# TheCacophonyProject/classifier-pipeline

Measured on AMD Instinct MI355X. Metric: CPTV frames/s end-to-end (track+classify) at 160x120, higher is better.
Workload: dtype u16/i32 track stage (f32 normalise, f64 gates); f32 crop/tile; f32 CNN (stride-1 3x3 convs of stages 2-4 (+ the stride-2 one): two fp16 planes per operand rounded to nearest (11 + 11 significand bits), power-of-two range scaling, 3 fp16 MFMAs per K step, device-side rerun in the exact split if an ac

## Files before the change

classifier-pipeline_amd/csrc/cpx_api.cpp:

```cpp
#include <hip/hip_runtime.h>

#include <algorithm>
#include <cmath>
#include <cstdio>
#include <cstdlib>
#include <cstring>
#include <new>
#include <string>
#include <vector>

#include "cpx_internal.h"
#include "cpx_schedule_core.h"

static_assert(sizeof(cpx_component) == 32, "cpx_component layout is part of the ABI");
static_assert(sizeof(cpx_frame_info) == 80, "cpx_frame_info layout is part of the ABI");
static_assert(sizeof(cpx_frame_meta) == 24, "cpx_frame_meta layout is part of the ABI");
static_assert(sizeof(cpx_config) == 48, "cpx_config layout is part of the ABI");
static_assert(sizeof(cpx_region_ref) == 24 && sizeof(cpx_track_limits) == 32 && sizeof(cpx_crop_req) == 32,
              "classification request layouts are part of the ABI");
static_assert(sizeof(cpx_filter_params) == 72 && sizeof(cpx_track_summary) == 120,
              "end-of-clip layouts are part of the ABI");
static_assert(sizeof(cpx_region) == 56, "cpx_region layout is part of the ABI");
static_assert(sizeof(cpx_track_record) == 32, "cpx_track_record layout is part of the ABI");
static_assert(sizeof(cpx_track_params) == 120, "cpx_track_params layout is part of the ABI");

namespace {

struct WsLayout {
  size_t bg, wsum, kcnt, filt, cstate, u8, carry, bgavg, big, total;
};

WsLayout ws_layout(const cpx_config& c, int B, bool need_filt_state) {
  const size_t P = (size_t)c.width * c.height;
  WsLayout l{};
  size_t off = 0;
  l.bg = off;
  off = align_up(off + (size_t)B * 2 * P * sizeof(uint16_t), 256);
  l.wsum = off;
  off = align_up(off + (size_t)B * P * sizeof(uint32_t), 256);
  l.kcnt = off;
  off = align_up(off + (size_t)B * P * sizeof(uint16_t), 256);
  l.filt = off;
  if (need_filt_state) off = align_up(off + (size_t)B * 2 * P * sizeof(float), 256);
  l.cstate = off;
  off = align_up(off + (size_t)B * sizeof(cpx::ClipState), 256);
  l.u8 = off;
  off = align_up(off + (size_t)B * 2 * P, 256);
  l.carry = off;
  off = align_up(off + (size_t)B * 2 * sizeof(cpx::FrameCarry), 256);
  l.bgavg = off;
  off = align_up(off + (size_t)B * sizeof(double), 256);
  l.big = off;
  if (c.max_components > cpx::track_lds_components())
    off = align_up(off + (size_t)B * 9 * c.max_components * sizeof(uint32_t), 256);
  l.total = off;
  return l;
}

int build_schedule(cpx_handle* h, const int32_t* clip_offsets, const cpx_frame_meta* meta, int B, cpx::Schedule* sc) {
  switch (cpx::schedule_build(clip_offsets, meta, B, h->cfg.max_frames, sc)) {
    case cpx::SchedError::EmptyClip: return fail(h, CPX_ERR_INVALID, "empty clip in batch");
    case cpx::SchedError::TooLong: return fail(h, CPX_ERR_INVALID, "clip longer than max_frames");
    case cpx::SchedError::Ok: break;
  }
  return CPX_OK;
}

int upload_schedule(cpx_handle* h, const cpx::Schedule& sc, int B, cpx::SchedLayout* sl) {
  const std::vector<int> flat = cpx::schedule_flatten(sc, B);
  *sl = cpx::SchedLayout::of(B, (int)sc.proc_idx.size());
  if (int rc = h->sched.grow(h, flat.size() * sizeof(int), "schedule hipMalloc")) return rc;
  CPX_HIP(h, hipMemcpyAsync(h->sched.p, flat.data(), flat.size() * sizeof(int), hipMemcpyHostToDevice, h->stream));
  CPX_HIP(h, hipStreamSynchronize(h->stream));
  return CPX_OK;
}

}

extern "C" {

int cpx_abi_version(void) { return CPX_ABI_VERSION; }

int cpx_create(int device_id, const cpx_config* cfg, cpx_handle** out) {
  if (!cfg || !out) return CPX_ERR_INVALID;
  *out = nullptr;
  int ndev = 0;
  if (hipGetDeviceCount(&ndev) != hipSuccess || ndev <= 0) return CPX_ERR_NO_DEVICE;
  if (device_id < 0 || device_id >= ndev) return CPX_ERR_INVALID;
  const int W = cfg->width, H = cfg->height;
  if (W <= 0 || H <= 0 || (W % 8) != 0 || W >= 192 || W * H > cpx::track_max_pixels() || H < 5 || W < 8)
    return CPX_ERR_UNSUPPORTED;
  if (cfg->edge_pixels < 0 || 2 * cfg->edge_pixels >= std::min(W, H) || cfg->window < 1 ||
      cfg->max_components < 1 || cfg->max_frames < 1 || cfg->max_frames > 65534)
    return CPX_ERR_INVALID;
  cpx_handle* h = new (std::nothrow) cpx_handle();
  if (!h) return CPX_ERR_NOMEM;
  h->device = device_id;
  h->cfg = *cfg;
  if (hipSetDevice(device_id) != hipSuccess || hipStreamCreateWithFlags(&h->stream, hipStreamNonBlocking) != hipSuccess ||
      hipStreamCreateWithFlags(&h->stream2, hipStreamNonBlocking) != hipSuccess ||
      hipEventCreateWithFlags(&h->ev_median, hipEventDisableTiming) != hipSuccess ||
      hipEventCreate(&h->ev0) != hipSuccess || hipEventCreate(&h->ev1) != hipSuccess) {
    cpx_destroy(h);
    return CPX_ERR_HIP;
  }
  h->wtab_len = 65536;
  h->wtab_host.resize(h->wtab_len);
  std::vector<double>& wt = h->wtab_host;
  double w = 0.0;
  for (int k = 0; k < h->wtab_len; ++k) {
    wt[k] = w;
    w = w + cfg->weight_add;
  }
  if (cfg->denoise) {
    if (!cpx::nlm_supported(W, H)) {
      cpx_destroy(h);
      return CPX_ERR_UNSUPPORTED;
    }
    const int fixed_point_mult = (int)(2147483647LL / (21 * 21 * 255));
    std::vector<int> lut(64, 0);
    for (int a2 = 0; a2 < 64; ++a2) {
      const double wv = std::exp(-((double)a2 * (64.0 / 49.0)) / 9.0);
      const double wr = std::nearbyint((double)fixed_point_mult * wv);
      lut[a2] = (wr < 0.001 * fixed_point_mult) ? 0 : (int)wr;
    }
    if (lut[63] != 0 || h->nlm_lut_dev.grow(h, 64 * sizeof(int), "NLM weight table allocation") ||
        hipMemcpy(h->nlm_lut_dev.p, lut.data(), 64 * sizeof(int), hipMemcpyHostToDevice) != hipSuccess) {
      cpx_destroy(h);
      return CPX_ERR_HIP;
    }
  }
  std::vector<uint32_t> thr(h->wtab_len);
  for (int k = 0; k < h->wtab_len; ++k) {
    const double wk = wt[k], m = std::nearbyint(wk);
    const bool exact = (wk == m), near = !exact && std::fabs(wk - m) < 1e-6;
    double hi = near ? m + 1.0 : std::floor(wk) + 1.0;
    if (!(hi >= 0.0)) hi = 0.0;
    if (hi > 536870912.0) hi = 536870912.0;
    thr[k] = 2u * (uint32_t)hi - (near ? 1u : 0u);
  }
  if (h->wthr_dev.grow(h, thr.size() * sizeof(uint32_t), "threshold table allocation") ||
      hipMemcpy(h->wthr_dev.p, thr.data(), thr.size() * sizeof(uint32_t), hipMemcpyHostToDevice) != hipSuccess) {
    cpx_destroy(h);
    return CPX_ERR_HIP;
  }
  if (h->wtab_dev.grow(h, wt.size() * sizeof(double), "weight table allocation") ||
      hipMemcpy(h->wtab_dev.p, wt.data(), wt.size() * sizeof(double), hipMemcpyHostToDevice) != hipSuccess ||
      cpx::frame_kernel_attr_setup() != 0) {
    cpx_destroy(h);
    return CPX_ERR_HIP;
  }
  if (const char* env = std::getenv("CPX_TRACK_PACKED_STATE")) h->packed_state_ok = std::atoi(env) != 0;
  if (const char* env = std::getenv("CPX_CNN_FUSE_CONV1")) h->fuse_conv1 = std::atoi(env) != 0;
  if (const char* env = std::getenv("CPX_TRACK_PER_STEP")) h->track_per_step = std::atoi(env) != 0;
  if (const char* env = std::getenv("CPX_CNN_FUSE_SHORTCUT")) h->fuse_shortcut = std::atoi(env) != 0;
  if (const char* env = std::getenv("CPX_CNN_SHORTCUT_FP16")) h->shortcut_fp16 = std::atoi(env) != 0;
  if (const char* env = std::getenv("CPX_CNN_BLOCK_FUSION")) h->block_fusion = std::min(std::max(std::atoi(env), 0), 2);
  if (const char* env = std::getenv("CPX_CNN_MATH")) {
    if (!std::strcmp(env, "f32")) h->cnn_math = CPX_CNN_MATH_F32;
    else if (!std::strcmp(env, "bf16x3")) h->cnn_math = CPX_CNN_MATH_BF16X3;
    else if (!std::strcmp(env, "bf16x2")) h->cnn_math = CPX_CNN_MATH_BF16X2;
    else if (!std::strcmp(env, "fp16x2")) h->cnn_math = CPX_CNN_MATH_FP16X2;
  }
  *out = h;
  return CPX_OK;
}

static void release_buffers(cpx_handle* h, bool all) {
  for (DeviceBuffer* b : {&h->ws, &h->ws_assoc, &h->bf3_scratch, &h->cnn_arena, &h->graph_arena, &h->ir_scratch}) b->release();
  if (!all) return;
  for (DeviceBuffer* b : {&h->sched, &h->wtab_dev, &h->wthr_dev, &h->nlm_lut_dev, &h->cnn_ovf, &h->ir_bitmap}) b->release();
}

void cpx_destroy(cpx_handle* h) {
  if (!h) return;
  hipSetDevice(h->device);
  if (h->stream) hipStreamSynchronize(h->stream);
  for (cpx_cnn* c : h->cnns) cnn_free(c);
  h->cnns.clear();
  for (cpx_mog2* m : h->mog2s) mog2_free(m);
  h->mog2s.clear();
  for (cpx_graph* g : h->graphs) graph_free(g);
  h->graphs.clear();
  release_buffers(h, true);
  for (auto& e : h->conv_events) {
    hipEventDestroy(e.e0);
    hipEventDestroy(e.e1);
  }
  if (h->stream2) {
    hipStreamSynchronize(h->stream2);
    hipStreamDestroy(h->stream2);
  }
  if (h->ev_median) hipEventDestroy(h->ev_median);
  if (h->ev0) hipEventDestroy(h->ev0);
  if (h->ev1) hipEventDestroy(h->ev1);
  if (h->stream) hipStreamDestroy(h->stream);
  delete h;
}

const char* cpx_last_error(const cpx_handle* h) { return h ? h->err.c_str() : "null handle"; }

void* cpx_stream(cpx_handle* h) { return h ? (void*)h->stream : nullptr; }

static int join_medians(cpx_handle* h) {
  if (h->medians_pending) {
    h->medians_pending = false;
    CPX_HIP(h, hipStreamWaitEvent(h->stream, h->ev_median, 0));
  }
  return CPX_OK;
}

int cpx_join_medians(cpx_handle* h) {
  if (!h) return CPX_ERR_INVALID;
  return join_medians(h);
}

int cpx_release_memory(cpx_handle* h) {
  if (!h) return CPX_ERR_INVALID;
  CPX_ENTER(h);
  if (int rc = join_medians(h)) return rc;
  CPX_HIP(h, hipStreamSynchronize(h->stream));
  CPX_HIP(h, hipStreamSynchronize(h->stream2));
  release_buffers(h, false);
  h->last_B = 0;
  h->state_packed = false;
  return CPX_OK;
}

int cpx_synchronize(cpx_handle* h) {
  if (!h) return CPX_ERR_INVALID;
  if (int rc = join_medians(h)) return rc;
  CPX_HIP(h, hipStreamSynchronize(h->stream));
  return CPX_OK;
}

size_t cpx_track_workspace_bytes(const cpx_handle* h, int B, int total_frames) {
  if (!h || B <= 0) return 0;
  (void)total_frames;
  return ws_layout(h->cfg, B, true).total;
}

static int unpack_state(cpx_handle* h) {
  if (h->state_packed && h->ws.p && h->last_B > 0) {
    const WsLayout lp = ws_layout(h->cfg, h->last_B, h->stream_filt_state);
    char* base = h->ws.as<char>();
    cpx::launch_unpack_state((uint32_t*)(base + lp.wsum), (uint16_t*)(base + lp.kcnt),
                             (size_t)h->last_B * h->cfg.width * h->cfg.height, h->stream);
    CPX_HIP(h, hipGetLastError());
  }
  h->state_packed = false;
  return CPX_OK;
}

static int track_run(cpx_handle* h, const uint16_t* frames_dev, const int32_t* clip_offsets,
                     const cpx_frame_meta* meta, int B, int n_prev, cpx_component* comps_dev,
                     cpx_frame_info* info_dev, int32_t* labels_dev, float* filtered_dev,
                     float* background_dev, int flags) {
  CPX_ENTER(h);
  if (flags & ~(CPX_TRACK_KEEP_BACKGROUND | CPX_TRACK_FREEZE_ON_FFC | CPX_TRACK_FREEZE_BACKGROUND | CPX_TRACK_DEFER_MEDIANS))
    return fail(h, CPX_ERR_INVALID, "track: unknown flag");
  if (int jrc = join_medians(h)) return jrc;
  const bool defer_medians = (flags & CPX_TRACK_DEFER_MEDIANS) != 0;
  const cpx_config& c = h->cfg;
  cpx::Schedule sc;
  int rc = build_schedule(h, clip_offsets, meta, B, &sc);
  if (rc != CPX_OK) return rc;
  const int total = sc.total, max_proc = sc.max_proc;
  const bool resume = n_prev > 0;
  const int t_begin = cpx::processed_before(meta, n_prev);
  const bool need_filt = (filtered_dev == nullptr);
  const WsLayout l = ws_layout(c, B, need_filt);
  if (resume && (l.total > h->ws.bytes || need_filt != h->stream_filt_state))
    return fail(h, CPX_ERR_INVALID, "cpx_track_frame: the stream's workspace is gone (optional outputs changed?)");
  const bool keep = !resume && (flags & CPX_TRACK_KEEP_BACKGROUND);
  if (keep) {
    const bool have_prev = h->ws.p && h->last_B == B && need_filt == h->stream_filt_state && l.total <= h->ws.bytes;
    for (int b = 0; b < B && !have_prev; ++b)
      if (!h->staged_bg.count(b)) {
        h->staged_bg.clear();
        return fail(h, CPX_ERR_INVALID, "CPX_TRACK_KEEP_BACKGROUND: no background state for a clip (previous call had another batch size, and nothing staged; staged states dropped)");
      }
  }
  for (const auto& kv : h->staged_bg)
    if (kv.first >= B) {
      h->staged_bg.clear();
      return fail(h, CPX_ERR_INVALID, "cpx_set_background: staged clip index outside the batch (staged states dropped)");
    }
  if (resume || keep) {
    if (int urc = unpack_state(h)) return urc;
  }
  h->state_packed = false;
  h->stream_filt_state = need_filt;
  h->last_B = B;
  struct StateGuard {
    cpx_handle* h;
    bool armed = true;
    ~StateGuard() {
      if (armed) {
        h->last_B = 0;
        h->state_packed = false;
      }
    }
  } guard{h};
  if ((rc = h->ws.grow(h, l.total, "workspace hipMalloc"))) return rc;
  cpx::SchedLayout sl;
  rc = upload_schedule(h, sc, B, &sl);
  if (rc != CPX_OK) return rc;

  cpx::TrackArgs a{};
// ... 611 lines not shown
```

classifier-pipeline_amd/csrc/cpx_api_cnn.cpp:

```cpp
#include <hip/hip_runtime.h>

#include <algorithm>
#include <cmath>
#include <cstdio>
#include <cstdlib>
#include <new>
#include <utility>
#include <vector>

#include "cpx_internal.h"

static_assert(sizeof(cpx_wrresnet_block) == 56 && sizeof(cpx_wrresnet_params) == 1560,
              "cpx_wrresnet_params layout is part of the ABI");

struct cpx_cnn {
  cpx_handle* h = nullptr;
  cpx_wrresnet_params p{};
  std::vector<std::pair<const float*, void*>> split;
  float act_scale[3][CPX_WRRESNET_MAX_BLOCKS][2];
  float res_bound[3] = {0.0f, 0.0f, 0.0f};
  float sc_xscale[3] = {0.0f, 0.0f, 0.0f};
  void* sc_img[3] = {nullptr, nullptr, nullptr};
  double sc_wmax[3] = {-1.0, -1.0, -1.0};
  cpx_cnn() {
    for (auto& st : act_scale)
      for (auto& b : st) b[0] = b[1] = 1.0f;
  }
  const void* split_of(const float* w) const {
    for (const auto& e : split)
      if (e.first == w) return e.second;
    return nullptr;
  }
};

void cnn_free(cpx_cnn* c) {
  for (auto& e : c->split) hipFree(e.second);
  for (void* img : c->sc_img)
    if (img) hipFree(img);
  delete c;
}

struct conv_fuse {
  const float* in = nullptr;
  const float* w = nullptr;
  const float* bias = nullptr;
  int H = 0, W = 0, cin = 0, stride = 1;
  const void* planes = nullptr;
  float xscale = 0.0f;
};

static bool split_math(const cpx_handle* h) { return h->cnn_math != CPX_CNN_MATH_F32; }
struct conv_half {
  float act_scale = 1.0f;
  bool keep_flag = false;
  int word = 0;
  bool out_planes = false;
  float out_act_scale = 1.0f;
  bool in_planes = false;
  bool rerun_only = false;
};
constexpr int OVF_WORDS = 2 + 3 * CPX_WRRESNET_MAX_BLOCKS;
static int ensure_ovf_word(cpx_handle* h) {
  if (h->cnn_ovf.p) return CPX_OK;
  if (int rc = h->cnn_ovf.grow(h, OVF_WORDS * sizeof(int), "cpx_conv2d: overflow word allocation failed")) return rc;
  CPX_HIP(h, hipMemsetAsync(h->cnn_ovf.p, 0, OVF_WORDS * sizeof(int), h->stream));
  return CPX_OK;
}
static cpx::ConvArgs conv_shape(int N, int H, int W, int Cin, int Cout, int groups, int ksize, int stride, int pad_same) {
  cpx::ConvArgs a{};
  a.N = N; a.H = H; a.W = W; a.Cin = Cin; a.Cout = Cout; a.groups = groups; a.ksize = ksize; a.stride = stride;
  if (pad_same) {
    a.Ho = (H + stride - 1) / stride;
    a.Wo = (W + stride - 1) / stride;
    a.pad_top = std::max((a.Ho - 1) * stride + ksize - H, 0) / 2;
    a.pad_left = std::max((a.Wo - 1) * stride + ksize - W, 0) / 2;
  } else {
    a.Ho = (H - ksize) / stride + 1;
    a.Wo = (W - ksize) / stride + 1;
  }
  return a;
}
static cpx::ConvArgs conv_describe(const cpx_conv_desc& d, const conv_fuse* fuse = nullptr) {
  cpx::ConvArgs a = conv_shape(d.N, d.H, d.W, d.Cin, d.Cout, d.groups, d.ksize, d.stride, d.pad_same);
  a.relu = d.relu;
  a.in = d.in_dev; a.out = d.out_dev; a.weights = d.weights_dev;
  a.in_scale = d.in_scale_dev; a.in_shift = d.in_shift_dev;
  a.out_scale = d.out_scale_dev; a.out_shift = d.out_shift_dev; a.residual = d.residual_dev;
  if (fuse) {
    a.sc_in = fuse->in; a.sc_w = fuse->w; a.sc_bias = fuse->bias;
    a.sc_H = fuse->H; a.sc_W = fuse->W; a.sc_cin = fuse->cin; a.sc_stride = fuse->stride;
    a.sc_planes = fuse->planes; a.sc_xscale = fuse->xscale;
  }
  return a;
}

class ConvTimer {
 public:
  ConvTimer(cpx_handle* h, bool on) : h_(h) {
    if (!on) return;
    ok_ = hipEventCreate(&ev_.e0) == hipSuccess && hipEventCreate(&ev_.e1) == hipSuccess &&
          hipEventRecord(ev_.e0, h->stream) == hipSuccess;
  }
  ~ConvTimer() {
    if (ev_.e0) hipEventDestroy(ev_.e0);
    if (ev_.e1) hipEventDestroy(ev_.e1);
  }
  ConvTimer(const ConvTimer&) = delete;
  ConvTimer& operator=(const ConvTimer&) = delete;
  bool ok() const { return ok_; }
  int commit(int key, double flops) {
    if (!ev_.e0) return CPX_OK;
    CPX_HIP(h_, hipEventRecord(ev_.e1, h_->stream));
    ev_.key = key;
    ev_.flops = flops;
    h_->conv_events.push_back(ev_);
    ev_ = {};
    return CPX_OK;
  }

 private:
  cpx_handle* h_;
  cpx_handle::ConvEv ev_{};
  bool ok_ = true;
};

enum class ConvRoute {
  Float32,
  Split,
  Fp16Pair,
  RerunOnly,
};

static int conv_run(cpx_handle* h, const cpx_conv_desc* d, const void* split_weights, const conv_fuse* fuse = nullptr,
                    const conv_half* hf = nullptr) {
  if (!h) return CPX_ERR_INVALID;
  if (!d || !d->in_dev || !d->out_dev || !d->weights_dev) return fail(h, CPX_ERR_INVALID, "cpx_conv2d: null argument");
  if (d->N < 1 || d->H < 1 || d->W < 1 || d->groups < 1 || d->Cin % d->groups || d->Cout % d->groups ||
      d->ksize < 1 || d->stride < 1 || (d->in_scale_dev == nullptr) != (d->in_shift_dev == nullptr))
    return fail(h, CPX_ERR_INVALID, "cpx_conv2d: bad descriptor");
  CPX_ENTER(h);
  if (!d->pad_same && (d->H < d->ksize || d->W < d->ksize)) return fail(h, CPX_ERR_INVALID, "cpx_conv2d: input smaller than kernel");
  cpx::ConvArgs a = conv_describe(*d, fuse);
  const bool split = split_math(h) && cpx::conv_bf3_supported(a);
  if (fuse && (!split || a.out_scale || a.residual))
    return fail(h, CPX_ERR_INVALID, "conv_run: shortcut fusion needs the split-operand kernel, no output scale, no residual");
  if (split) a.planes = h->cnn_math == CPX_CNN_MATH_BF16X2 ? 2 : 3;
  const conv_half bare;
  const conv_half& k = hf ? *hf : bare;
  const bool fp16 = split && h->cnn_math == CPX_CNN_MATH_FP16X2;
  const bool aliased = a.out == a.residual || a.out == a.in;
  const bool half = fp16 && cpx::conv_bf3_two_planes(a) && !aliased;
  const bool planes_out = fp16 && k.out_planes;
  const ConvRoute route = k.rerun_only ? ConvRoute::RerunOnly
                          : !split ? ConvRoute::Float32
                          : (half || planes_out) ? ConvRoute::Fp16Pair
                                                 : ConvRoute::Split;
  ConvTimer timer(h, h->conv_timing && route != ConvRoute::RerunOnly);
  if (!timer.ok()) return fail(h, CPX_ERR_HIP, "cpx_conv2d: event creation failed");
  int* word = nullptr;
  if (route == ConvRoute::Fp16Pair || route == ConvRoute::RerunOnly) {
    if (int rc = ensure_ovf_word(h)) return rc;
    if (!k.keep_flag) CPX_HIP(h, hipMemsetAsync(h->cnn_ovf.p, 0, sizeof(int), h->stream));
    word = h->cnn_ovf.as<int>() + k.word;
  }
  if (split && !split_weights) {
    if (int rc = h->bf3_scratch.grow(h, cpx::conv_bf3_weight_bytes(a), "cpx_conv2d: weight scratch allocation failed"))
      return rc;
    cpx::launch_split_weights(a, h->bf3_scratch.p, h->stream);
    split_weights = h->bf3_scratch.p;
  }
  int rc = 0;
  if (route == ConvRoute::Fp16Pair) {
    cpx::ConvArgs first = a;
    if (half) {
      first.planes = 2;
      first.half = 1;
      first.act_scale = k.act_scale;
      first.act_unscale = 1.0f / first.act_scale;
      first.in_planes = k.in_planes;
    }
    first.ovf = word;
    if (planes_out) {
      first.out_planes = 1;
      first.out_act_scale = k.out_act_scale;
    }
    rc = cpx::launch_conv_bf3(first, split_weights, h->stream);
  }
  a.guard = word;
  if (split) {
    if (rc == 0) rc = cpx::launch_conv_bf3(a, split_weights, h->stream);
    if (rc == -3) {
      if (fuse) return fail(h, CPX_ERR_UNSUPPORTED, "conv_run: batch too large for the fused-shortcut kernel (split the call)");
      rc = cpx::launch_conv(a, h->stream);
    }
  } else {
    rc = cpx::launch_conv(a, h->stream);
  }
  if (int trc = timer.commit((a.Cin / a.groups) * 10000 + (a.Cout / a.groups) * 10 + a.stride + (a.ksize == 1 ? 5 : 0),
                             2.0 * a.N * a.Ho * a.Wo * a.Cout * (double)(a.Cin / a.groups) * a.ksize * a.ksize))
    return trc;
  if (rc == -2) return fail(h, CPX_ERR_UNSUPPORTED, "cpx_conv2d: no kernel for this (channels per group, stride, kernel size)");
  if (rc != 0) return fail(h, CPX_ERR_HIP, "cpx_conv2d: kernel configuration failed");
  CPX_HIP(h, hipGetLastError());
  return CPX_OK;
}

static bool conv_can_fuse(const cpx_handle* h, int f, int groups) {
  return split_math(h) && cpx::conv_bf3_supported(conv_shape(0, 0, 0, f, f, groups, 3, 1, 1));
}

enum class BlockForm {
  OneLaunch,
  PlanesPair,
  Separate,
};
enum class Shortcut {
  Identity,
  FusedIntoSecond,
  OwnLaunch,
};
enum class Conv1 {
  NotHere,
  InFront,
  InsideBlock,
};
enum class Fusion { None, Block, BlockAndConv1 };

struct BlockPlan {
  int k, st, d;
  int stride, H, W, Ho, Wo, c_in, f;
  int word;
  BlockForm form;
  Shortcut shortcut;
  bool shortcut_fp16;
  Conv1 conv1;
};

struct Forward {
  cpx_cnn* cnn;
  cpx_handle* h;
  const float* in;
  int N, H, W;
  float *act[2], *mid, *sc;
};

static cpx_conv_desc layer_desc(const Forward& fw, const float* in, float* out, const float* w, int H, int W, int cin, int cout,
                                int ksize, int stride, int same, int relu) {
  cpx_conv_desc d{};
  d.N = fw.N; d.H = H; d.W = W; d.Cin = cin; d.Cout = cout; d.groups = fw.cnn->p.groups; d.ksize = ksize; d.stride = stride;
  d.pad_same = same; d.relu = relu;
  d.in_dev = in; d.out_dev = out; d.weights_dev = w;
  return d;
}

struct BlockLayers {
  cpx_conv_desc a, sc, b;
  conv_fuse fuse;
};
static BlockLayers block_layers(const Forward& fw, const BlockPlan& bp) {
  const cpx_wrresnet_params& p = fw.cnn->p;
  const cpx_wrresnet_block& b = p.block[bp.st][bp.d];
  const float* cur = fw.act[bp.k & 1];
  BlockLayers l{};
  l.a = layer_desc(fw, cur, fw.mid, b.wa, bp.H, bp.W, bp.c_in, bp.f, 3, bp.stride, 1, 1);
  l.a.in_scale_dev = b.in_scale; l.a.in_shift_dev = b.in_shift; l.a.out_scale_dev = b.a_scale; l.a.out_shift_dev = b.a_shift;
  l.sc = layer_desc(fw, cur, fw.sc, p.shortcut_w[bp.st], bp.H, bp.W, bp.c_in, bp.f, 1, bp.stride, 0, 0);
  l.sc.out_shift_dev = p.shortcut_b[bp.st];
  l.fuse.in = cur; l.fuse.w = p.shortcut_w[bp.st]; l.fuse.bias = p.shortcut_b[bp.st];
  l.fuse.H = bp.H; l.fuse.W = bp.W; l.fuse.cin = bp.c_in; l.fuse.stride = bp.stride;
  if (bp.shortcut_fp16) {
    l.fuse.planes = fw.cnn->sc_img[bp.st];
    l.fuse.xscale = fw.cnn->sc_xscale[bp.st];
  }
  l.b = layer_desc(fw, fw.mid, fw.act[(bp.k + 1) & 1], b.wb, bp.Ho, bp.Wo, bp.f, bp.f, 3, 1, 1, 1);
  l.b.out_shift_dev = b.bb;
  l.b.residual_dev = bp.shortcut == Shortcut::Identity ? cur : bp.shortcut == Shortcut::OwnLaunch ? fw.sc : nullptr;
  return l;
}
static void block32_args(const Forward& fw, const BlockPlan& bp, cpx::ConvArgs* ca, cpx::ConvArgs* cb) {
  const BlockLayers l = block_layers(fw, bp);
  *ca = conv_describe(l.a);
  *cb = conv_describe(l.b, bp.shortcut == Shortcut::FusedIntoSecond ? &l.fuse : nullptr);
  cpx::ConvArgs* both[2] = {ca, cb};
  for (int i = 0; i < 2; ++i) {
    both[i]->planes = 2;
    both[i]->half = 1;
    both[i]->ovf = fw.h->cnn_ovf.as<int>() + bp.word;
    both[i]->act_scale = fw.cnn->act_scale[bp.st][bp.d][i];
    both[i]->act_unscale = 1.0f / both[i]->act_scale;
  }
  if (bp.conv1 == Conv1::InsideBlock) {
    ca->c1_in = fw.in; ca->c1_w = fw.cnn->p.conv1_w; ca->c1_b = fw.cnn->p.conv1_b;
  }
}

static BlockPlan plan_block(const Forward& fw, int k, int H, int W, Fusion most) {
  const cpx_handle* h = fw.h;
  const cpx_cnn* cnn = fw.cnn;
  const cpx_wrresnet_params& p = cnn->p;
  const int g = p.groups;
  BlockPlan bp{};
  bp.k = k; bp.st = k / p.blocks_per_stage; bp.d = k % p.blocks_per_stage;
  const cpx_wrresnet_block& b = p.block[bp.st][bp.d];
  bp.stride = bp.d == 0 ? bp.st + 1 : 1;
  bp.c_in = p.filters[bp.d == 0 ? bp.st : bp.st + 1];
  bp.f = p.filters[bp.st + 1];
  const cpx::ConvArgs first = conv_shape(fw.N, H, W, bp.c_in, bp.f, g, 3, bp.stride, 1);
  const cpx::ConvArgs second = conv_shape(fw.N, first.Ho, first.Wo, bp.f, bp.f, g, 3, 1, 1);
  bp.H = H; bp.W = W; bp.Ho = first.Ho; bp.Wo = first.Wo;
  bp.word = 2 + k;
  const bool fp16 = h->cnn_math == CPX_CNN_MATH_FP16X2, whole_groups = bp.c_in % g == 0 && bp.f % g == 0;
  bp.shortcut = bp.d != 0 ? Shortcut::Identity
                : (h->fuse_shortcut && conv_can_fuse(h, bp.f, g) && (bp.c_in / g) % 4 == 0) ? Shortcut::FusedIntoSecond
                                                                                          : Shortcut::OwnLaunch;
  bp.shortcut_fp16 = bp.shortcut == Shortcut::FusedIntoSecond && fp16 && h->shortcut_fp16 && cnn->sc_xscale[bp.st] > 0.0f &&
                     cnn->sc_img[bp.st] != nullptr;
  const bool first8 = bp.d == 0 && bp.stride == 1 && bp.c_in / g == 8 && h->block_fusion >= 2 && h->fuse_shortcut;
  bool one_launch = most != Fusion::None && fp16 && h->block_fusion && bp.stride == 1 &&
                    ((bp.d != 0 && bp.c_in == bp.f) || first8) && b.in_scale && cnn->split_of(b.wa) && cnn->split_of(b.wb) &&
                    whole_groups;
  if (one_launch) {
    cpx::ConvArgs ca, cb;
    block32_args(fw, bp, &ca, &cb);
    one_launch = cpx::conv_block32_supported(ca, cb);
  }
  const bool c1_inside = one_launch && most == Fusion::BlockAndConv1 && k == 0 && first8 && h->fuse_conv1 && g == 2 &&
                         p.in_channels == 2 && p.filters[0] == 16;
  bp.conv1 = k != 0 ? Conv1::NotHere : c1_inside ? Conv1::InsideBlock : Conv1::InFront;
  const bool planes = fp16 && whole_groups && cpx::conv_bf3_can_store_planes(first) && cpx::conv_bf3_two_planes(second) &&
                      cpx::conv_bf3_can_load_planes(second);
  bp.form = one_launch ? BlockForm::OneLaunch : planes ? BlockForm::PlanesPair : BlockForm::Separate;
  return bp;
}

static int run_layer(const Forward& fw, const cpx_conv_desc& d, const conv_half& hf, const conv_fuse* fuse = nullptr) {
  return conv_run(fw.h, &d, fw.cnn->split_of(d.weights_dev), fuse, &hf);
}
static conv_half forward_half(int word, bool rerun_only) {
  conv_half hf;
  hf.keep_flag = true;
  hf.word = word;
  hf.rerun_only = rerun_only;
  return hf;
}

static int run_conv1(const Forward& fw, const conv_half& hf) {
  const cpx_wrresnet_params& p = fw.cnn->p;
  cpx_conv_desc d = layer_desc(fw, fw.in, fw.act[0], p.conv1_w, fw.H, fw.W, p.in_channels, p.filters[0], 3, 1, 1, 0);
  d.out_shift_dev = p.conv1_b;
  return run_layer(fw, d, hf);
}

static int run_layers(const Forward& fw, const BlockPlan& bp, bool planes, bool rerun_only) {
  const BlockLayers l = block_layers(fw, bp);
  const float* act_scale = fw.cnn->act_scale[bp.st][bp.d];
  const conv_half hf = forward_half(bp.word, rerun_only);
  conv_half ha = hf, hb = hf;
  ha.act_scale = act_scale[0];
  ha.out_planes = planes;
  ha.out_act_scale = act_scale[1];
  hb.act_scale = act_scale[1];
  hb.in_planes = planes;
  if (int rc = run_layer(fw, l.a, ha)) return rc;
  if (bp.shortcut == Shortcut::OwnLaunch)
    if (int rc = run_layer(fw, l.sc, hf)) return rc;
  return run_layer(fw, l.b, hb, bp.shortcut == Shortcut::FusedIntoSecond ? &l.fuse : nullptr);
}

static int run_one_launch(const Forward& fw, const BlockPlan& bp, int* declined) {
  cpx_handle* h = fw.h;
  const cpx_wrresnet_params& p = fw.cnn->p;
  const cpx_wrresnet_block& b = p.block[bp.st][bp.d];
  const int g = p.groups;
  cpx::ConvArgs ca, cb;
  block32_args(fw, bp, &ca, &cb);
  ConvTimer timer(h, h->conv_timing);
  if (!timer.ok()) return fail(h, CPX_ERR_HIP, "cpx_cnn_forward: event creation failed");
  *declined = cpx::launch_conv_block32(ca, cb, fw.cnn->split_of(b.wa), fw.cnn->split_of(b.wb), h->stream);
  if (*declined) return CPX_OK;
  double flops = 2.0 * fw.N * bp.H * bp.W * bp.f * ((double)(bp.c_in / g) + (double)(bp.f / g)) * 9;
  if (bp.conv1 == Conv1::InsideBlock) flops += 2.0 * fw.N * bp.H * bp.W * bp.c_in * (double)(p.in_channels / g) * 9;
  if (int rc = timer.commit((bp.c_in / g) * 10000 + 32 * 10 + 4, flops)) return rc;
  if (bp.conv1 == Conv1::InsideBlock)
    if (int rc = run_conv1(fw, forward_half(bp.word, true))) return rc;
  return run_layers(fw, bp, false, true);
}

static int downgrade(const Forward& fw, BlockPlan* bp, int declined) {
  if (bp->conv1 == Conv1::InsideBlock) {
    *bp = plan_block(fw, bp->k, bp->H, bp->W, Fusion::Block);
    return run_conv1(fw, forward_half(0, false));
  }
  if (declined != -2 && declined != -3) return fail(fw.h, CPX_ERR_HIP, "cpx_cnn_forward: block kernel configuration failed");
  *bp = plan_block(fw, bp->k, bp->H, bp->W, Fusion::None);
  return CPX_OK;
}

static int run_block(const Forward& fw, BlockPlan bp) {
  if (bp.conv1 == Conv1::InFront)
    if (int rc = run_conv1(fw, forward_half(0, false))) return rc;
  while (bp.form == BlockForm::OneLaunch) {
    int declined = 0;
    if (int rc = run_one_launch(fw, bp, &declined)) return rc;
    if (!declined) return CPX_OK;
    if (int rc = downgrade(fw, &bp, declined)) return rc;
  }
  return run_layers(fw, bp, bp.form == BlockForm::PlanesPair, false);
}

static int update_shortcut_images(cpx_cnn* cnn) {
  cpx_handle* h = cnn->h;
  const cpx_wrresnet_params& p = cnn->p;
  CPX_ENTER(h);
  for (int st = 0; st < 3; ++st) {
    cnn->sc_xscale[st] = 0.0f;
    const int g = p.groups, c_in = p.filters[st], f = p.filters[st + 1];
    if (!(cnn->res_bound[st] > 0.0f) || c_in % g || f % g) continue;
    cpx::ConvArgs second = conv_shape(0, 0, 0, f, f, g, 3, 1, 1);
    second.weights = p.block[st][0].wb;
    const void* wimg = cnn->split_of(second.weights);
    if (!wimg || !cpx::conv_shortcut_planes_layer(second, c_in / g)) continue;
    const int cin_g = c_in / g, cout_g = f / g;
    const float* w_scale_dev = cpx::conv_bf3_weight_scales(second, wimg);
    if (cnn->sc_wmax[st] < 0.0) {
      std::vector<float> ws((size_t)f), w((size_t)g * cin_g * cout_g);
      CPX_HIP(h, hipStreamSynchronize(h->stream));
      CPX_HIP(h, hipMemcpy(ws.data(), w_scale_dev, ws.size() * sizeof(float), hipMemcpyDeviceToHost));
      CPX_HIP(h, hipMemcpy(w.data(), p.shortcut_w[st], w.size() * sizeof(float), hipMemcpyDeviceToHost));
      double m = 0.0;
      for (int gi = 0; gi < g; ++gi)
        for (int k = 0; k < cin_g; ++k)
          for (int c = 0; c < cout_g; ++c)
            m = std::max(m, std::fabs((double)w[((size_t)gi * cin_g + k) * cout_g + c]) * ws[gi * cout_g + c]);
      cnn->sc_wmax[st] = m;
    }
    const float act_scale = cnn->act_scale[st][0][1];
    const double wmax = cnn->sc_wmax[st] * act_scale;
    float sx = 0.0f;
    if (!cpx_cnn_shortcut_scale(cnn->res_bound[st], (float)wmax, &sx)) continue;
    if (!cnn->sc_img[st] && hipMalloc(&cnn->sc_img[st], cpx::conv_shortcut_image_bytes(g, cin_g, cout_g)) != hipSuccess) {
      (void)hipGetLastError();
      cnn->sc_img[st] = nullptr;
      return fail(h, CPX_ERR_NOMEM, "cpx_cnn_set_residual_bounds: shortcut image allocation failed");
    }
    cpx::launch_split_shortcut(p.shortcut_w[st], cnn->sc_img[st], g, cin_g, cout_g, w_scale_dev, act_scale / sx, h->stream);
    CPX_HIP(h, hipGetLastError());
    cnn->sc_xscale[st] = sx;
  }
  return CPX_OK;
}

static int cnn_forward(cpx_cnn* cnn, const float* in_dev, int N, int H, int W, float* logits_dev, float* probs_dev,
                       float* const* taps, int* ovf_out) {
  cpx_handle* h = cnn->h;
  CPX_ENTER(h);
  const cpx_wrresnet_params& p = cnn->p;
  if (h->cnn_math == CPX_CNN_MATH_FP16X2) {
    const int rco = ensure_ovf_word(h);
    if (rco != CPX_OK) return rco;
    CPX_HIP(h, hipMemsetAsync(h->cnn_ovf.as<int>() + 2, 0, (OVF_WORDS - 2) * sizeof(int), h->stream));
  }
  size_t biggest = 0;
  {
    int hh = H, ww = W;
    biggest = (size_t)N * hh * ww * p.filters[0];
    for (int st = 0; st < 3; ++st) {
      const int s = st + 1;
      hh = (hh + s - 1) / s;
      ww = (ww + s - 1) / s;
      biggest = std::max(biggest, (size_t)N * hh * ww * p.filters[st + 1]);
    }
  }
  biggest = align_up(biggest, 64);
  if (int rc = h->cnn_arena.grow(h, 4 * biggest * sizeof(float), "cpx_cnn_forward: activation hipMalloc")) return rc;
  float* const arena = h->cnn_arena.as<float>();
  const Forward fw{cnn, h, in_dev, N, H, W, {arena, arena + biggest}, arena + 2 * biggest, arena + 3 * biggest};
  const int n_blocks = 3 * p.blocks_per_stage;
  BlockPlan plan[3 * CPX_WRRESNET_MAX_BLOCKS];
  int hh = H, ww = W;
  for (int k = 0; k < n_blocks; ++k) {
    plan[k] = plan_block(fw, k, hh, ww, Fusion::BlockAndConv1);
    hh = plan[k].Ho;
    ww = plan[k].Wo;
  }
  for (int k = 0; k < n_blocks; ++k) {
    if (int brc = run_block(fw, plan[k])) return brc;
    if (taps)
      CPX_HIP(h, hipMemcpyAsync(taps[k], fw.act[(k + 1) & 1], (size_t)N * plan[k].Ho * plan[k].Wo * plan[k].f * sizeof(float),
                                hipMemcpyDeviceToDevice, h->stream));
  }
  const float* cur = fw.act[n_blocks & 1];
  const int c_in = plan[n_blocks - 1].f;
  cpx_head_desc hd{};
  hd.N = N; hd.HW = hh * ww; hd.C = c_in; hd.L = p.n_labels;
  hd.n_hidden = p.n_hidden;
  hd.activation = p.activation;
  for (int k = 0; k < p.n_hidden; ++k) {
    hd.hidden_sizes[k] = p.hidden_sizes[k];
    hd.hidden_w_dev[k] = p.hidden_w[k];
    hd.hidden_b_dev[k] = p.hidden_b[k];
  }
  hd.in_dev = cur; hd.bn_scale_dev = p.final_scale; hd.bn_shift_dev = p.final_shift;
  hd.dense_w_dev = p.dense_w; hd.dense_b_dev = p.dense_b; hd.logits_dev = logits_dev; hd.probs_dev = probs_dev;
  int rc = cpx_cnn_head_ex(h, &hd);
  if (rc == CPX_OK && h->cnn_math == CPX_CNN_MATH_FP16X2)
    cpx::launch_count_overflow(h->cnn_ovf.as<int>(), 3 * p.blocks_per_stage, h->stream);
  if (rc == CPX_OK && ovf_out) {
    const size_t bytes = (size_t)3 * p.blocks_per_stage * sizeof(int);
    if (h->cnn_math == CPX_CNN_MATH_FP16X2)
      CPX_HIP(h, hipMemcpyAsync(ovf_out, h->cnn_ovf.as<int>() + 2, bytes, hipMemcpyDeviceToDevice, h->stream));
    else
      CPX_HIP(h, hipMemsetAsync(ovf_out, 0, bytes, h->stream));
  }
  if (rc == CPX_OK && h->cnn_math == CPX_CNN_MATH_FP16X2 && std::getenv("CPX_CNN_DEBUG_OVF")) {
    int words[OVF_WORDS];
    if (hipStreamSynchronize(h->stream) == hipSuccess &&
        hipMemcpy(words, h->cnn_ovf.p, sizeof(words), hipMemcpyDeviceToHost) == hipSuccess && words[0]) {
      std::fprintf(stderr, "cpx_cnn_forward: N = %d, fp16 overflow in blocks", N);
      for (int k = 0; k < 3 * p.blocks_per_stage; ++k)
        if (words[2 + k]) std::fprintf(stderr, " %d.%d", k / p.blocks_per_stage + 2, k % p.blocks_per_stage);
      std::fprintf(stderr, "\n");
    }
  }
  return rc;
}

extern "C" {

int cpx_conv2d(cpx_handle* h, const cpx_conv_desc* d) { return conv_run(h, d, nullptr); }

int cpx_set_cnn_math(cpx_handle* h, int mode) {
  if (!h) return CPX_ERR_INVALID;
  if (mode != CPX_CNN_MATH_F32 && mode != CPX_CNN_MATH_BF16X3 && mode != CPX_CNN_MATH_BF16X2 && mode != CPX_CNN_MATH_FP16X2)
    return fail(h, CPX_ERR_INVALID, "cpx_set_cnn_math: unknown mode");
  h->cnn_math = mode;
  return CPX_OK;
}
int cpx_get_cnn_math(const cpx_handle* h) { return h ? h->cnn_math : CPX_ERR_INVALID; }

int cpx_cnn_overflow_forwards(cpx_handle* h, int* count, int reset) {
  if (!h) return CPX_ERR_INVALID;
  if (!count) return fail(h, CPX_ERR_INVALID, "cpx_cnn_overflow_forwards: null argument");
  CPX_ENTER(h);
  *count = 0;
  if (!h->cnn_ovf.p) return CPX_OK;
  CPX_HIP(h, hipStreamSynchronize(h->stream));
  CPX_HIP(h, hipMemcpy(count, h->cnn_ovf.as<int>() + 1, sizeof(int), hipMemcpyDeviceToHost));
  if (reset) CPX_HIP(h, hipMemset(h->cnn_ovf.as<int>() + 1, 0, sizeof(int)));
  return CPX_OK;
}

int cpx_cnn_last_overflow(cpx_handle* h, int* overflowed) {
  if (!h) return CPX_ERR_INVALID;
  if (!overflowed) return fail(h, CPX_ERR_INVALID, "cpx_cnn_last_overflow: null argument");
  CPX_ENTER(h);
  *overflowed = 0;
  if (!h->cnn_ovf.p) return CPX_OK;
  CPX_HIP(h, hipStreamSynchronize(h->stream));
  CPX_HIP(h, hipMemcpy(overflowed, h->cnn_ovf.p, sizeof(int), hipMemcpyDeviceToHost));
  return CPX_OK;
}

int cpx_cnn_head_ex(cpx_handle* h, const cpx_head_desc* d) {
  if (!h) return CPX_ERR_INVALID;
  if (!d || !d->in_dev || !d->bn_scale_dev || !d->bn_shift_dev || !d->dense_w_dev || !d->dense_b_dev || !d->logits_dev ||
      d->N < 1 || d->HW < 1 || d->C < 1 || d->L < 1 || d->C > 8192 || d->L > 8192 || d->n_hidden < 0 ||
      d->n_hidden > CPX_HEAD_MAX_HIDDEN || (d->activation != CPX_HEAD_SIGMOID && d->activation != CPX_HEAD_SOFTMAX))
    return fail(h, CPX_ERR_INVALID, "cpx_cnn_head: bad argument");
  CPX_ENTER(h);
  cpx::HeadArgs a{};
  a.N = d->N; a.HW = d->HW; a.C = d->C; a.L = d->L;
  a.n_hidden = d->n_hidden;
  a.activation = d->activation;
  for (int k = 0; k < d->n_hidden; ++k) {
    if (!d->hidden_w_dev[k] || !d->hidden_b_dev[k] || d->hidden_sizes[k] < 1 || d->hidden_sizes[k] > 2048)
      return fail(h, CPX_ERR_INVALID, "cpx_cnn_head: bad hidden layer");
    a.hidden_sizes[k] = d->hidden_sizes[k];
    a.hidden_w[k] = d->hidden_w_dev[k];
    a.hidden_b[k] = d->hidden_b_dev[k];
  }
  a.in = d->in_dev; a.bn_scale = d->bn_scale_dev; a.bn_shift = d->bn_shift_dev;
  a.dense_w = d->dense_w_dev; a.dense_b = d->dense_b_dev; a.logits = d->logits_dev; a.probs = d->probs_dev;
  cpx::launch_head(a, h->stream);
  CPX_HIP(h, hipGetLastError());
  return CPX_OK;
}

int cpx_cnn_head(cpx_handle* h, const float* in_dev, int N, int HW, int C, const float* bn_scale_dev,
                 const float* bn_shift_dev, const float* dense_w_dev, const float* dense_b_dev, int L,
                 float* logits_dev, float* probs_dev) {
  if (!h) return CPX_ERR_INVALID;
  cpx_head_desc d{};
  d.N = N; d.HW = HW; d.C = C; d.L = L;
  d.n_hidden = 0;
  d.activation = CPX_HEAD_SIGMOID;
  d.in_dev = in_dev; d.bn_scale_dev = bn_scale_dev; d.bn_shift_dev = bn_shift_dev;
  d.dense_w_dev = dense_w_dev; d.dense_b_dev = dense_b_dev; d.logits_dev = logits_dev; d.probs_dev = probs_dev;
  return cpx_cnn_head_ex(h, &d);
}

int cpx_conv_timing_enable(cpx_handle* h, int enable) {
  if (!h) return CPX_ERR_INVALID;
  for (auto& e : h->conv_events) {
    hipEventDestroy(e.e0);
    hipEventDestroy(e.e1);
  }
  h->conv_events.clear();
  h->conv_timing = enable != 0;
  return CPX_OK;
}

int cpx_conv_timing_report(cpx_handle* h, cpx_conv_timing* out, int cap, int* n_out) {
  if (!h || !out || !n_out || cap < 1) return CPX_ERR_INVALID;
  CPX_HIP(h, hipStreamSynchronize(h->stream));
  int n = 0;
  for (auto& e : h->conv_events) {
    float ms = 0.f;
    CPX_HIP(h, hipEventElapsedTime(&ms, e.e0, e.e1));
    int i = 0;
    for (; i < n; ++i)
      if (out[i].key == e.key) break;
    if (i == n) {
      if (n == cap) return fail(h, CPX_ERR_OVERFLOW, "cpx_conv_timing_report: more kernel variants than capacity");
      out[n].key = e.key;
      out[n].launches = 0;
      out[n].total_ms = 0.0;
      out[n].flops = 0.0;
      n += 1;
    }
    out[i].launches += 1;
    out[i].total_ms += ms;
    out[i].flops += e.flops;
  }
  *n_out = n;
  return CPX_OK;
}
// ... 133 lines not shown
```

classifier-pipeline_amd/csrc/cpx_cnn_bf3.hip:

```cpp
#include <hip/hip_runtime.h>

#include <algorithm>
#include <cstdlib>
#include <type_traits>

#include "cpx_conv_layout_core.h"
#include "cpx_kernels.h"

namespace cpx {

namespace {

typedef float f32x16 __attribute__((ext_vector_type(16)));
typedef __bf16 bf16x8 __attribute__((ext_vector_type(8)));
typedef __bf16 bf16x2 __attribute__((ext_vector_type(2)));
typedef unsigned u32x4 __attribute__((ext_vector_type(4)));
typedef float f32x4 __attribute__((ext_vector_type(4)));

__device__ __forceinline__ unsigned pack2(float a, float b) {
  bf16x2 v = {(__bf16)a, (__bf16)b};
  return __builtin_bit_cast(unsigned, v);
}
template <typename T>
__device__ __forceinline__ const T* at_off(const T* base, unsigned bytes) {
// ... 372 lines not shown
      __builtin_amdgcn_fence(__ATOMIC_ACQUIRE, "wavefront");
      if (res_n) {
#pragma unroll
        for (int it = 0; it < 4; ++it) {
          const int f = it * 64 + lane;
          const int i = f >> 3, c4 = f & 7;
          const int oy = oy0 + (wset + m * WSETS) * TB + WR * wave + i / TW, ox = ox0 + i % TW;
          if (oy < a.Ho && ox < a.Wo) {
            float4 v = *reinterpret_cast<const float4*>(s_tile + i * 32 + 4 * c4);
            const int o = (int)pix_off(oy, ox, a.Wo, a.Cout) + ch0 + t * 32 + 4 * c4;
            const float4 rv = *reinterpret_cast<const float4*>(at_off(res_n, (unsigned)o << 2));
            v.x += rv.x; v.y += rv.y; v.z += rv.z; v.w += rv.w;
            if (a.relu) {
              v.x = relu_bits(v.x); v.y = relu_bits(v.y); v.z = relu_bits(v.z); v.w = relu_bits(v.w);
            }
            *reinterpret_cast<float4*>(at_off(out_n, (unsigned)o << 2)) = v;
          }
        }
      } else if (full_tile) {
        const unsigned lb = (pix_off(oy0 + (wset + m * WSETS) * TB + WR * wave, ox0 + (lane >> 3), a.Wo, a.Cout) +
                             (unsigned)(ch0 + t * 32 + 4 * (lane & 7))) << 2;
#pragma unroll
        for (int it = 0; it < 4; ++it) {
          float4 v = *reinterpret_cast<const float4*>(s_tile + (it * 64 + lane) * 4);
          const unsigned ub = (unsigned)((((it * 8) / TW) * a.Wo + ((it * 8) % TW)) * a.Cout) << 2;
          if (a.relu) {
            v.x = relu_bits(v.x); v.y = relu_bits(v.y); v.z = relu_bits(v.z); v.w = relu_bits(v.w);
          }
          if (a.out_planes) {
            const f32x4 vv = {v.x, v.y, v.z, v.w};
            if (max_abs4(vv) > F16_MAX) atomicOr(a.ovf, 1);
            *reinterpret_cast<u32x4*>(at_off(out_n, lb + ub)) = planes_of(vv);
          } else {
            *reinterpret_cast<float4*>(at_off(out_n, lb + ub)) = v;
          }
        }
      } else {
#pragma unroll
        for (int it = 0; it < 4; ++it) {
          const int f = it * 64 + lane;
          const int i = f >> 3, c4 = f & 7;
          const int oy = oy0 + (wset + m * WSETS) * TB + WR * wave + i / TW, ox = ox0 + i % TW;
          if (oy < a.Ho && ox < a.Wo) {
            float4 v = *reinterpret_cast<const float4*>(s_tile + i * 32 + 4 * c4);
            const int o = (int)pix_off(oy, ox, a.Wo, a.Cout) + ch0 + t * 32 + 4 * c4;
            if (a.relu) {
              v.x = relu_bits(v.x); v.y = relu_bits(v.y); v.z = relu_bits(v.z); v.w = relu_bits(v.w);
            }
            if (a.out_planes) {
              const f32x4 vv = {v.x, v.y, v.z, v.w};
              if (max_abs4(vv) > F16_MAX) atomicOr(a.ovf, 1);
              *reinterpret_cast<u32x4*>(at_off(out_n, (unsigned)o << 2)) = planes_of(vv);
            } else {
              *reinterpret_cast<float4*>(at_off(out_n, (unsigned)o << 2)) = v;
            }
          }
        }
      }
      if (m + 1 < NTM || t + 1 < NTN) {
        __builtin_amdgcn_fence(__ATOMIC_RELEASE, "wavefront");
        __builtin_amdgcn_wave_barrier();
        __builtin_amdgcn_fence(__ATOMIC_ACQUIRE, "wavefront");
      }
    }
  }
  BF3_TILE_LOOP_END
}

template <int NTN, int NPXC, int PL, bool H = false, bool PERSIST = false, int CT = 256, bool SC = false>
__global__ __launch_bounds__(CT) void conv_bf3flat_kernel(ConvArgs a, const uint4* __restrict__ wimg, TileDiv td) {
  constexpr int KS = 3, BAND = CT / 2;
  constexpr int COGW = 32 * NTN;
  static_assert(!H || PL == 2, "fp16 planes come in twos");
  static_assert(!SC || (H && !PERSIST && CT == 256 && 4 * 2 * 2 * BAND + 4 * 2 * 2 * COGW <= 2 * PL * NPXC + 18 * PL * COGW),
                "the shortcut's planes reuse the LDS of the patch and the weights");
  extern __shared__ __attribute__((aligned(16))) uint4 lds4[];
  BF3_ENTRY_GUARD(H)
  uint4* s_patch = lds4;
  uint4* s_w = lds4 + 2 * PL * NPXC;

  const int tid = threadIdx.x, lane = tid & 63, wave = tid >> 6;
  BF3_TILE_LOOP_BEGIN
  int bid = bid0;
  if (!PERSIST && (gridDim.x & 7) == 0) bid = (bid & 7) * (gridDim.x >> 3) + (bid >> 3);
  const int cin_g = a.Cin / a.groups, cout_g = a.Cout / a.groups;
  int q = div_magic(bid, td.m_nsplit);
  const int ns = bid - q * td.nsplit;
  bid = q;
  q = div_magic(bid, td.m_tx);
  const int ti = bid - q * td.tiles_x;
  const int n = q;
  const int g = blockIdx.y;
  const int M = a.Ho * a.Wo;
  const int p0 = ti * BAND;
  const int y_first = p0 / a.Wo, y_last = min(p0 + BAND - 1, M - 1) / a.Wo;
  const int PW = a.W + 2, PH = y_last - y_first + 3;
  const int npx = PH * PW;
  const int iy0 = y_first - a.pad_top, ix0 = -a.pad_left;
  const float* in_n = a.in + (size_t)n * a.H * a.W * a.Cin + (size_t)g * cin_g;
  const int nchunks = cin_g / KC;
  const uint4* wg = wimg + (size_t)g * nchunks * (18 * PL) * cout_g + (size_t)ns * COGW;

  const bool res_in_acc = a.residual != nullptr && a.out_scale == nullptr;
  f32x16 acc[NTN];
  if (res_in_acc) {
    const float* res_n = a.residual + (size_t)n * M * a.Cout + (g * cout_g + ns * COGW);
    const int rcol = lane & 31;
#pragma unroll
    for (int t = 0; t < NTN; ++t) {
      const float rs = H ? a.w_scale[g * cout_g + ns * COGW + t * 32 + rcol] * a.act_scale : 1.0f;
#pragma unroll
      for (int r = 0; r < 16; ++r) {
        const int i = (r & 3) + 8 * (r >> 2) + 4 * (lane >> 5);
        acc[t][r] = *at_off(res_n, (__umul24((unsigned)min(p0 + wave * 32 + i, M - 1), (unsigned)a.Cout) + (unsigned)(t * 32 + rcol)) << 2);
        if (H) acc[t][r] *= rs;
      }
    }
  } else {
#pragma unroll
    for (int t = 0; t < NTN; ++t)
#pragma unroll
      for (int r = 0; r < 16; ++r) acc[t][r] = 0.0f;
  }

  const int kh = lane >> 5;
  const int pl = min(p0 + wave * 32 + (lane & 31), M - 1);
  const int ly = pl / a.Wo, lx = pl - ly * a.Wo;
  const int a_base = kh * NPXC + (ly - y_first) * PW + lx;
  const int b_base = kh * COGW + (lane & 31);

  constexpr int NP = (2 * NPXC + CT - 1) / CT;
  constexpr int NW = 18 * PL * COGW;
  constexpr int NWI = (NW + CT - 1) / CT;
  const int my_h = tid & 1;
  int item_py[NP], item_px[NP], item_e[NP];
#pragma unroll
  for (int i = 0; i < NP; ++i) {
    const int item = min(tid + i * CT, 2 * npx - 1);
    const int px = item >> 1;
    item_py[i] = px / PW;
    item_px[i] = px - item_py[i] * PW;
    item_e[i] = my_h * NPXC + px;
  }
  f32x4 pre_p[NP][2];
  u32x4 pre_w[NWI];
  f32x4 psc[2], psh[2];
  for (int cc = -1; cc < nchunks; ++cc) {
    if (cc >= 0) {
      float vmax = 0.0f;
#pragma unroll
      for (int i = 0; i < NP; ++i) {
        const int iy = iy0 + item_py[i], ix = ix0 + item_px[i];
        const bool inside = iy >= 0 && iy < a.H && ix >= 0 && ix < a.W;
        float v[8];
#pragma unroll
        for (int j = 0; j < 8; ++j) v[j] = pre_p[i][j >> 2][j & 3];
        if (a.in_scale) {
#pragma unroll
          for (int j = 0; j < 8; ++j) v[j] = fmaxf(__fmaf_rn(v[j], psc[j >> 2][j & 3], psh[j >> 2][j & 3]), 0.0f);
        } else if (H) {
#pragma unroll
          for (int j = 0; j < 8; ++j) v[j] *= a.act_scale;
        }
#pragma unroll
        for (int j = 0; j < 8; ++j) v[j] = inside ? v[j] : 0.0f;
        if (H) {
#pragma unroll
          for (int j = 0; j < 8; j += 2) vmax = fmaxf(fmaxf(fabsf(v[j]), fabsf(v[j + 1])), vmax);
        }
        unsigned q0[4], q1[4], q2[4];
#pragma unroll
        for (int j = 0; j < 4; ++j) {
          if (PL == 3) split_pair(v[2 * j], v[2 * j + 1], q0[j], q1[j], q2[j]);
          else split2<H>(v[2 * j], v[2 * j + 1], q0[j], q1[j]);
        }
        u32x4* sp4 = reinterpret_cast<u32x4*>(s_patch);
        sp4[0 * 2 * NPXC + item_e[i]] = u32x4{q0[0], q0[1], q0[2], q0[3]};
        sp4[1 * 2 * NPXC + item_e[i]] = u32x4{q1[0], q1[1], q1[2], q1[3]};
        if (PL == 3) sp4[2 * 2 * NPXC + item_e[i]] = u32x4{q2[0], q2[1], q2[2], q2[3]};
      }
#pragma unroll
      for (int i = 0; i < NWI; ++i) {
        const int item = tid + i * CT;
        if (item < NW) reinterpret_cast<u32x4*>(s_w)[item] = pre_w[i];
      }
      if (H && vmax > F16_MAX) atomicOr(a.ovf, 1);
      __syncthreads();
    }
    if (cc + 1 < nchunks) {
      const int cn = (cc + 1) * KC;
      {
        const int ch = g * cin_g + cn;
        const float* scp = a.in_scale ? a.in_scale + ch : reinterpret_cast<const float*>(wimg);
        const float* shp = a.in_scale ? a.in_shift + ch : reinterpret_cast<const float*>(wimg);
        unsigned hoff = (unsigned)my_h << 5;
        asm volatile("" : "+v"(hoff));
        psc[0] = *reinterpret_cast<const f32x4*>(at_off(scp, hoff));
        psc[1] = *reinterpret_cast<const f32x4*>(at_off(scp, hoff + 16));
        psh[0] = *reinterpret_cast<const f32x4*>(at_off(shp, hoff));
        psh[1] = *reinterpret_cast<const f32x4*>(at_off(shp, hoff + 16));
        if (H) {
#pragma unroll
          for (int k = 0; k < 2; ++k) {
            psc[k] *= a.act_scale;
            psh[k] *= a.act_scale;
          }
        }
      }
#pragma unroll
      for (int i = 0; i < NP; ++i) {
        const int cy = min(max(iy0 + item_py[i], 0), a.H - 1), cx = min(max(ix0 + item_px[i], 0), a.W - 1);
        const unsigned soff = (pix_off(cy, cx, a.W, a.Cin) + (unsigned)(cn + 8 * my_h)) << 2;
        pre_p[i][0] = *reinterpret_cast<const f32x4*>(at_off(in_n, soff));
        pre_p[i][1] = *reinterpret_cast<const f32x4*>(at_off(in_n, soff + 16));
      }
      const u32x4* wc = reinterpret_cast<const u32x4*>(wg + (size_t)(cc + 1) * (18 * PL) * cout_g);
#pragma unroll
      for (int i = 0; i < NWI; ++i) {
        const int item = min(tid + i * CT, NW - 1);
        const int pth = item / COGW, col = item - pth * COGW;
        unsigned woff = (unsigned)(pth * cout_g + col) << 4;
        asm volatile("" : "+v"(woff));
        pre_w[i] = *at_off(wc, woff);
      }
    }
    if (cc >= 0) {
#pragma unroll
      for (int tap = 0; tap < KS * KS; ++tap) {
        const int ky = tap / KS, kx = tap - ky * KS;
        u32x4 av[PL], bv[NTN][PL];
#pragma unroll
        for (int p = 0; p < PL; ++p) {
          av[p] = __builtin_bit_cast(u32x4, s_patch[p * 2 * NPXC + a_base + ky * PW + kx]);
#pragma unroll
          for (int t = 0; t < NTN; ++t)
            bv[t][p] = __builtin_bit_cast(u32x4, s_w[(p * 9 + tap) * 2 * COGW + b_base + t * 32]);
        }
#pragma unroll
        for (int t = 0; t < NTN; ++t) {
          if (PL == 3) {
            acc[t] = mfma32<false>(av[1], bv[t][1], acc[t]);
            acc[t] = mfma32<false>(av[0], bv[t][PL - 1], acc[t]);
            acc[t] = mfma32<false>(av[PL - 1], bv[t][0], acc[t]);
          }
          acc[t] = mfma32<H>(av[0], bv[t][1], acc[t]);
          acc[t] = mfma32<H>(av[1], bv[t][0], acc[t]);
          acc[t] = mfma32<H>(av[0], bv[t][0], acc[t]);
        }
      }
      __syncthreads();
    }
  }

  if constexpr (SC) {
    uint4* s_x = lds4;
    uint4* s_scw = lds4 + 4 * 2 * 2 * BAND;
    {
      const int sp = min(p0 + (tid >> 1), M - 1);
      const int sy = sp / a.Wo, sxp = sp - sy * a.Wo;
      const float* src = a.sc_in + (((size_t)n * a.sc_H + sy * a.sc_stride) * a.sc_W + sxp * a.sc_stride) * a.sc_cin + g * 64 + 8 * my_h;
      f32x4 xv[4][2];
#pragma unroll
      for (int c = 0; c < 4; ++c) {
        xv[c][0] = *reinterpret_cast<const f32x4*>(src + 16 * c);
        xv[c][1] = *reinterpret_cast<const f32x4*>(src + 16 * c + 4);
      }
      u32x4 wv[4];
      const u32x4* scw = reinterpret_cast<const u32x4*>(a.sc_planes) + (size_t)g * 16 * cout_g + ns * COGW;
#pragma unroll
      for (int c = 0; c < 4; ++c) {
        const int col = tid & (COGW - 1), hh = (tid / COGW) & 1, pp = (tid / (2 * COGW)) & 1, j = 2 * c + hh;
        wv[c] = scw[(size_t)(((j >> 2) * 2 + pp) * 4 + (j & 3)) * cout_g + col];
      }
      float vmax = 0.0f;
#pragma unroll
      for (int c = 0; c < 4; ++c) {
        float v[8];
#pragma unroll
        for (int j = 0; j < 8; ++j) v[j] = xv[c][j >> 2][j & 3] * a.sc_xscale;
#pragma unroll
        for (int j = 0; j < 8; j += 2) vmax = fmaxf(fmaxf(fabsf(v[j]), fabsf(v[j + 1])), vmax);
        unsigned q0[4], q1[4];
#pragma unroll
        for (int j = 0; j < 4; ++j) split2<true>(v[2 * j], v[2 * j + 1], q0[j], q1[j]);
        u32x4* sx4 = reinterpret_cast<u32x4*>(s_x);
        sx4[((c * 2 + 0) * 2 + my_h) * BAND + (tid >> 1)] = u32x4{q0[0], q0[1], q0[2], q0[3]};
        sx4[((c * 2 + 1) * 2 + my_h) * BAND + (tid >> 1)] = u32x4{q1[0], q1[1], q1[2], q1[3]};
        reinterpret_cast<u32x4*>(s_scw)[c * (2 * 2 * COGW) + tid] = wv[c];
      }
      if (!(vmax <= F16_MAX)) atomicOr(a.ovf, 1);
    }
    __syncthreads();
#pragma unroll
    for (int c = 0; c < 4; ++c) {
      u32x4 av[2], bv[NTN][2];
#pragma unroll
      for (int p = 0; p < 2; ++p) {
        av[p] = __builtin_bit_cast(u32x4, s_x[((c * 2 + p) * 2 + kh) * BAND + wave * 32 + (lane & 31)]);
#pragma unroll
        for (int t = 0; t < NTN; ++t) bv[t][p] = __builtin_bit_cast(u32x4, s_scw[((c * 2 + p) * 2 + kh) * COGW + (lane & 31) + t * 32]);
      }
#pragma unroll
      for (int t = 0; t < NTN; ++t) {
        acc[t] = mfma32<true>(av[0], bv[t][1], acc[t]);
        acc[t] = mfma32<true>(av[1], bv[t][0], acc[t]);
        acc[t] = mfma32<true>(av[0], bv[t][0], acc[t]);
      }
    }
    __syncthreads();
  } else if (a.sc_in) {
    const int sc_cg = a.sc_cin / a.groups;
    const float* wsc = a.sc_w + (size_t)g * sc_cg * cout_g + ns * COGW + (lane & 31);
    const float* psc_in = a.sc_in + (((size_t)n * a.sc_H + ly * a.sc_stride) * a.sc_W + lx * a.sc_stride) * a.sc_cin +
                          g * sc_cg + kh;
    float ss[NTN];
#pragma unroll
    for (int t = 0; t < NTN; ++t) ss[t] = H ? a.w_scale[g * cout_g + ns * COGW + t * 32 + (lane & 31)] * a.act_scale : 1.0f;
    for (int k2 = 0; k2 < sc_cg; k2 += 2) {
      const float av = psc_in[k2];
#pragma unroll
      for (int t = 0; t < NTN; ++t) {
        float wv = wsc[(size_t)(k2 + kh) * cout_g + t * 32];
        if (H) wv *= ss[t];
        acc[t] = __builtin_amdgcn_mfma_f32_32x32x2f32(av, wv, acc[t], 0, 0, 0);
      }
    }
  }

  float* out_n = a.out + (size_t)n * M * a.Cout;
  const float* res_n = (a.residual && !res_in_acc) ? a.residual + (size_t)n * M * a.Cout : nullptr;
  float* s_tile = reinterpret_cast<float*>(lds4) + wave * (32 * 32);
  const int ch0 = g * cout_g + ns * COGW;
#pragma unroll
  for (int t = 0; t < NTN; ++t) {
    const int ch = ch0 + t * 32 + (lane & 31);
    float os = a.out_scale ? a.out_scale[ch] : 1.0f;
    if (H) os *= a.w_unscale[ch] * a.act_unscale;
    const float ob = (a.out_shift ? a.out_shift[ch] : 0.0f) + (a.sc_in && a.sc_bias ? a.sc_bias[ch] : 0.0f);
#pragma unroll
    for (int r = 0; r < 16; ++r) {
      const int i = (r & 3) + 8 * (r >> 2) + 4 * (lane >> 5);
      s_tile[i * 32 + (lane & 31)] = acc[t][r] * os + ob;
    }
    __builtin_amdgcn_fence(__ATOMIC_RELEASE, "wavefront");
    __builtin_amdgcn_wave_barrier();
    __builtin_amdgcn_fence(__ATOMIC_ACQUIRE, "wavefront");
    if (res_n) {
#pragma unroll
      for (int it = 0; it < 4; ++it) {
        const int f = it * 64 + lane;
        const int i = f >> 3, c4 = f & 7;
        const int p = p0 + wave * 32 + i;
        if (p < M) {
          f32x4 v = *reinterpret_cast<const f32x4*>(s_tile + i * 32 + 4 * c4);
          const int o = (int)__umul24((unsigned)p, (unsigned)a.Cout) + ch0 + t * 32 + 4 * c4;
          v += *reinterpret_cast<const f32x4*>(at_off(res_n, (unsigned)o << 2));
          if (a.relu) {
            v.x = relu_bits(v.x); v.y = relu_bits(v.y); v.z = relu_bits(v.z); v.w = relu_bits(v.w);
          }
          *reinterpret_cast<f32x4*>(at_off(out_n, (unsigned)o << 2)) = v;
        }
      }
    } else {
#pragma unroll
      for (int it = 0; it < 4; ++it) {
        const int f = it * 64 + lane;
        const int i = f >> 3, c4 = f & 7;
        const int p = p0 + wave * 32 + i;
        if (p < M) {
          f32x4 v = *reinterpret_cast<const f32x4*>(s_tile + i * 32 + 4 * c4);
          const int o = (int)__umul24((unsigned)p, (unsigned)a.Cout) + ch0 + t * 32 + 4 * c4;
          if (a.relu) {
            v.x = relu_bits(v.x); v.y = relu_bits(v.y); v.z = relu_bits(v.z); v.w = relu_bits(v.w);
          }
          *reinterpret_cast<f32x4*>(at_off(out_n, (unsigned)o << 2)) = v;
        }
      }
    }
    if (t + 1 < NTN) {
      __builtin_amdgcn_fence(__ATOMIC_RELEASE, "wavefront");
      __builtin_amdgcn_wave_barrier();
      __builtin_amdgcn_fence(__ATOMIC_ACQUIRE, "wavefront");
    }
  }
  BF3_TILE_LOOP_END
}

constexpr int KW = 32;
constexpr int W_TW = 16, W_TH = 16, W_PW = 18, W_NPX = 18 * 18;
constexpr int W_NPXP = 326;
constexpr int w_patch_entries(int planes) { return planes * 2 * W_NPXP * 2; }
constexpr int w_rows_resident(int planes) { return planes == 2 ? 3 : 1; }
constexpr int w_wsub_entries(int planes) { return w_rows_resident(planes) * planes * 3 * 4 * 32; }
template <bool WALK, bool LDSBN, int NH, int NG, int PL, bool H = false, bool PERSIST = false>
__global__ __launch_bounds__(512) __attribute__((amdgpu_waves_per_eu(4, 4))) void conv_bf3w_kernel(ConvArgs a, const uint4* __restrict__ wimg, TileDiv td) {
  static_assert(NG == 1 || (!WALK && !LDSBN && NH == 1), "the group walk is built for the one-slice, one-tile form");
  static_assert(PL == 2 || PL == 3, "two or three bf16 planes per operand");
  static_assert(!H || (PL == 2 && LDSBN), "fp16 planes come in twos (and with the BatchNorm parameters in LDS)");
  BF3_ENTRY_GUARD(H)
  constexpr int WR = w_rows_resident(PL);
  constexpr int W_PATCH = PL * 2 * W_NPXP * 2;
  constexpr int W_WROW = PL * 3 * 4 * 32;
  constexpr int W_WSUB = WR * W_WROW;
  constexpr int CT = 512;
  constexpr bool LAUNDER = WALK || NH > 1 || NG > 1 || PL == 2;
  extern __shared__ __attribute__((aligned(16))) uint4 lds4[];
  uint4* s_patch = lds4;
  uint4* s_w = lds4 + W_PATCH;

  const int tid = threadIdx.x, lane = tid & 63, wave = tid >> 6, i16 = lane & 15, q = lane >> 4;
  BF3_TILE_LOOP_BEGIN
  int bid = bid0;
  if (!PERSIST && (gridDim.x & 7) == 0) bid = (bid & 7) * (gridDim.x >> 3) + (bid >> 3);
  const int cin_g = a.Cin / a.groups, cout_g = a.Cout / a.groups;
  int qd = div_magic(bid, td.m_nsplit);
  const int ns = bid - qd * td.nsplit;
  bid = qd;
  qd = div_magic(bid, td.m_tx);
  const int txr = bid - qd * td.tiles_x;
  bid = qd;
  qd = div_magic(bid, td.m_ty);
  const int tyi = bid - qd * td.tiles_y;
  const int n = qd;
  const int g0 = blockIdx.y * NG;
  const int oy0 = tyi * W_TH;
  const int iy0 = oy0 - a.pad_top;
  const int run = WALK ? td.run : 1;
  const int tx_end = WALK ? min((txr + 1) * run, (a.Wo + W_TW - 1) / W_TW) : txr + 1;
  const float* in_n = a.in + (size_t)n * a.H * a.W * a.Cin;
  const int nch = cin_g / KW;
  const uint4* wg = wimg + (size_t)ns * (32 * NH);
  const int a_base = ((q >> 1) * W_NPXP + (2 * wave) * W_PW + i16) * 2 + (q & 1);
  const int b_base = q * 32 + i16;
  constexpr int NITEM = W_NPX * 8;
  constexpr int NP = (NITEM + CT - 1) / CT;
  constexpr int NWI = (W_WSUB + CT - 1) / CT;
  const int my_q8 = tid & 7;
  const int st_e2_0 = ((my_q8 >> 2) * W_NPXP + (tid >> 3)) * 4 + (my_q8 & 3);
  u32x4 pre_p[NP];
  u32x4 pre_w[NWI];
  f32x4* s_bn = reinterpret_cast<f32x4*>(lds4 + W_PATCH + W_WSUB);
#pragma clang diagnostic push
#pragma clang diagnostic ignored "-Wuninitialized"
  f32x4 psc_r, psh_r;
  if (LDSBN && a.in_scale) {
    if (tid < cin_g) {
      reinterpret_cast<float*>(s_bn)[tid] = a.in_scale[g0 * cin_g + tid] * (H ? a.act_scale : 1.0f);
      reinterpret_cast<float*>(s_bn)[cin_g + tid] = a.in_shift[g0 * cin_g + tid] * (H ? a.act_scale : 1.0f);
    }
    __syncthreads();
  }
#define BF3W_ISSUE_W(G_, C_, R_, HF_)                                                                     \
  {                                                                                                       \
    const uint4* wc = wg + (size_t)((((G_) * nch + (C_)) * 3 + (R_)) * (12 * PL)) * cout_g + (HF_) * 32;  \
    unsigned woff = (__umul24((unsigned)(tid >> 5), (unsigned)cout_g) + (unsigned)(tid & 31)) << 4;       \
    if (LAUNDER) asm volatile("" : "+v"(woff));                                                           \
    _Pragma("unroll") for (int i = 0; i < NWI; ++i) {                                                     \
       \
      const unsigned wo = (i == NWI - 1 && (W_WSUB % CT) != 0) ? (tid < (W_WSUB % CT) ? woff + ((unsigned)(16 * i * cout_g) << 4) : woff) : woff + ((unsigned)(16 * i * cout_g) << 4); \
      pre_w[i] = *at_off(reinterpret_cast<const u32x4*>(wc), wo);                                         \
    }                                                                                                     \
  }
#define BF3W_ISSUE_P(G_, C_, IX0_)                                                                        \
  {                                                                                                       \
    int t8 = tid >> 3;                                                                                    \
    if (LAUNDER) asm volatile("" : "+v"(t8));                                                             \
    int my_q8 = tid & 7;                                                                                  \
    if (LAUNDER) asm volatile("" : "+v"(my_q8));                                                          \
    if (!LDSBN) {                                                                                         \
      const int ch = (G_) * cin_g + (C_) * KW;                                                            \
      const float* scp = a.in_scale ? a.in_scale + ch : reinterpret_cast<const float*>(wimg);             \
      const float* shp = a.in_scale ? a.in_shift + ch : reinterpret_cast<const float*>(wimg);             \
      unsigned qoff = (unsigned)my_q8 << 4;                                                               \
      asm volatile("" : "+v"(qoff));                                                                      \
      psc_r = *reinterpret_cast<const f32x4*>(at_off(scp, qoff));                                         \
      psh_r = *reinterpret_cast<const f32x4*>(at_off(shp, qoff));                                         \
    }                                                                                                     \
    const unsigned coff = (unsigned)((G_) * cin_g + (C_) * KW + 4 * my_q8);                               \
    _Pragma("unroll") for (int i = 0; i < NP; ++i) {                                                      \
      const int px = min(t8 + 64 * i, W_NPX - 1);                                                         \
                                            \
      const int py = (int)(__umul24((unsigned)px, 3641u) >> 16), pxx = __mul24(py, -W_PW) + px;           \
      const int cy = min(max(iy0 + py, 0), a.H - 1), cx = min(max((IX0_) + pxx, 0), a.W - 1);             \
      pre_p[i] = *reinterpret_cast<const u32x4*>(at_off(in_n, (pix_off(cy, cx, a.W, a.Cin) + coff) << 2)); \
    }                                                                                                     \
  }
  BF3W_ISSUE_W(g0, 0, 0, 0)
  BF3W_ISSUE_P(g0, 0, txr * run * W_TW - a.pad_left)
  for (int txi = txr * run; txi < tx_end; ++txi) {
  const int ox0 = txi * W_TW, ix0 = ox0 - a.pad_left;
  const bool interior = iy0 >= 0 && iy0 + 18 <= a.H && ix0 >= 0 && ix0 + 18 <= a.W;
  const bool full_tile = oy0 + W_TH <= a.Ho && ox0 + W_TW <= a.Wo;

  int ch_l;
  unsigned opix[2];
  bool ovalid[2];
  auto out_pixels = [&](const int g) __attribute__((always_inline)) {
    int t = tid;
    if (LAUNDER) asm volatile("" : "+v"(t));
    const int i16_ = t & 15, q_ = (t >> 4) & 3, wave_ = t >> 6;
// ... 794 lines not shown
  }
}

__global__ __launch_bounds__(256) void weight_scales_kernel(const float* __restrict__ w, float* __restrict__ wscale,
                                                            float* __restrict__ wunscale, int groups, int rows, int cout_g) {
  const int idx = blockIdx.x * blockDim.x + threadIdx.x;
  if (idx >= groups * cout_g) return;
  const int g = idx / cout_g, col = idx - g * cout_g;
  float m = 0.0f;
  for (int r = 0; r < rows; ++r) m = fmaxf(m, fabsf(w[((size_t)g * rows + r) * cout_g + col]));
  int e = 0;
  if (m > 0.0f && m < 3.0e38f) (void)frexpf(m, &e);
  else e = 4;
  const int kw = min(max(4 - e, -100), 100);
  wscale[idx] = ldexpf(1.0f, kw);
  wunscale[idx] = ldexpf(1.0f, -kw);
}

__global__ __launch_bounds__(256) void split_weights8h_kernel(const float* __restrict__ w, uint4* __restrict__ out, int groups,
                                                              const float* __restrict__ wscale) {
  const size_t total = (size_t)groups * 3 * 4 * 32;
  for (size_t idx = (size_t)blockIdx.x * blockDim.x + threadIdx.x; idx < total; idx += (size_t)gridDim.x * blockDim.x) {
    const int col = (int)(idx & 31), qq = (int)((idx >> 5) & 3), t = (int)((idx >> 7) % 3), g = (int)(idx / 384);
    const int tap = 4 * t + qq;
    const float ws = wscale[g * 32 + col];
    float v[8];
#pragma unroll
    for (int j = 0; j < 8; ++j) v[j] = tap < 9 ? w[(((size_t)g * 9 + tap) * 8 + j) * 32 + col] * ws : 0.0f;
    uint4 p0, p1;
    split_pair2_h(v[0], v[1], p0.x, p1.x);
    split_pair2_h(v[2], v[3], p0.y, p1.y);
    split_pair2_h(v[4], v[5], p0.z, p1.z);
    split_pair2_h(v[6], v[7], p0.w, p1.w);
    const size_t base = (size_t)g * B8_WIMG;
    out[base + (size_t)(t * 2 + 0) * 128 + qq * 32 + col] = p0;
    out[base + (size_t)(t * 2 + 1) * 128 + qq * 32 + col] = p1;
  }
}

__global__ __launch_bounds__(256) void split_weights_kernel(const float* __restrict__ w, uint4* __restrict__ out, int groups,
                                                            int cin_g, int cout_g, int planes, const float* __restrict__ wscale) {
  const int nchunks = cin_g / KC;
  const size_t total = (size_t)groups * nchunks * 9 * 2 * cout_g;
  for (size_t idx = (size_t)blockIdx.x * blockDim.x + threadIdx.x; idx < total; idx += (size_t)gridDim.x * blockDim.x) {
    size_t r = idx;
    const int col = (int)(r % cout_g);
    r /= cout_g;
    const int h = (int)(r & 1);
    r >>= 1;
    const int tap = (int)(r % 9);
    r /= 9;
    const int chunk = (int)(r % nchunks);
    const int g = (int)(r / nchunks);
    float v[8];
#pragma unroll
    for (int j = 0; j < 8; ++j)
      v[j] = w[(((size_t)g * 9 + tap) * cin_g + chunk * KC + 8 * h + j) * cout_g + col];
    uint4 p0, p1, p2;
    if (wscale) {
      const float ws = wscale[g * cout_g + col];
      split_pair2_h(v[0] * ws, v[1] * ws, p0.x, p1.x);
      split_pair2_h(v[2] * ws, v[3] * ws, p0.y, p1.y);
      split_pair2_h(v[4] * ws, v[5] * ws, p0.z, p1.z);
      split_pair2_h(v[6] * ws, v[7] * ws, p0.w, p1.w);
    } else if (planes == 3) {
      split_pair(v[0], v[1], p0.x, p1.x, p2.x);
      split_pair(v[2], v[3], p0.y, p1.y, p2.y);
      split_pair(v[4], v[5], p0.z, p1.z, p2.z);
      split_pair(v[6], v[7], p0.w, p1.w, p2.w);
    } else {
      split_pair2(v[0], v[1], p0.x, p1.x);
      split_pair2(v[2], v[3], p0.y, p1.y);
      split_pair2(v[4], v[5], p0.z, p1.z);
      split_pair2(v[6], v[7], p0.w, p1.w);
    }
    const size_t base = ((size_t)g * nchunks + chunk) * (18 * planes) * cout_g;
    out[base + ((size_t)(0 * 9 + tap) * 2 + h) * cout_g + col] = p0;
    out[base + ((size_t)(1 * 9 + tap) * 2 + h) * cout_g + col] = p1;
    if (planes == 3) out[base + ((size_t)(2 * 9 + tap) * 2 + h) * cout_g + col] = p2;
  }
}

__global__ __launch_bounds__(256) void split_weights32_kernel(const float* __restrict__ w, uint4* __restrict__ out, int groups,
                                                              int cin_g, int cout_g, int planes, const float* __restrict__ wscale) {
  const int nch = cin_g / KW;
  const size_t total = (size_t)groups * nch * 9 * 4 * cout_g;
  for (size_t idx = (size_t)blockIdx.x * blockDim.x + threadIdx.x; idx < total; idx += (size_t)gridDim.x * blockDim.x) {
    size_t r = idx;
    const int col = (int)(r % cout_g);
    r /= cout_g;
    const int qq = (int)(r & 3);
    r >>= 2;
    const int kx = (int)(r % 3);
    r /= 3;
    const int ky = (int)(r % 3);
    r /= 3;
    const int chunk = (int)(r % nch);
    const int g = (int)(r / nch);
    float v[8];
#pragma unroll
    for (int j = 0; j < 8; ++j)
      v[j] = w[(((size_t)g * 9 + ky * 3 + kx) * cin_g + chunk * KW + 8 * qq + j) * cout_g + col];
    uint4 p0, p1, p2;
    if (wscale) {
      const float ws = wscale[g * cout_g + col];
      split_pair2_h(v[0] * ws, v[1] * ws, p0.x, p1.x);
      split_pair2_h(v[2] * ws, v[3] * ws, p0.y, p1.y);
      split_pair2_h(v[4] * ws, v[5] * ws, p0.z, p1.z);
      split_pair2_h(v[6] * ws, v[7] * ws, p0.w, p1.w);
    } else if (planes == 3) {
      split_pair(v[0], v[1], p0.x, p1.x, p2.x);
      split_pair(v[2], v[3], p0.y, p1.y, p2.y);
      split_pair(v[4], v[5], p0.z, p1.z, p2.z);
      split_pair(v[6], v[7], p0.w, p1.w, p2.w);
    } else {
      split_pair2(v[0], v[1], p0.x, p1.x);
      split_pair2(v[2], v[3], p0.y, p1.y);
      split_pair2(v[4], v[5], p0.z, p1.z);
      split_pair2(v[6], v[7], p0.w, p1.w);
    }
    const size_t base = (((size_t)g * nch + chunk) * 3 + ky) * (12 * planes) * cout_g;
    out[base + ((size_t)(0 * 3 + kx) * 4 + qq) * cout_g + col] = p0;
    out[base + ((size_t)(1 * 3 + kx) * 4 + qq) * cout_g + col] = p1;
    if (planes == 3) out[base + ((size_t)(2 * 3 + kx) * 4 + qq) * cout_g + col] = p2;
  }
}

template <int NH, int PL, bool H = false>
static int launch_bf3w_t(const ConvArgs& a, const uint4* wimg, hipStream_t s) {
  const size_t lds = (size_t)(w_patch_entries(PL) + w_wsub_entries(PL)) * 16 + (size_t)(a.Cin / a.groups) * 8;
  static bool lds_ready[64], lds_ready_p[64];
  constexpr bool LDSBN = NH > 1 || PL == 2;
  if (!cpx_dyn_lds_ready(reinterpret_cast<const void*>(conv_bf3w_kernel<false, LDSBN, NH, 1, PL, H>), lds_ready, 160 * 1024 - 1024)) return -1;
  TileDiv td{};
  td.run = 1;
  if (const int rc = fill_tiles(td, (a.Wo + W_TW - 1) / W_TW, (a.Ho + W_TH - 1) / W_TH, a.N, (a.Cout / a.groups) / (32 * NH), TILES_PER_LAUNCH)) return rc;
  const long long blocks = td.total;
  if constexpr (PL == 3 && !H) if (a.guard != nullptr) {
    if (!cpx_dyn_lds_ready(reinterpret_cast<const void*>(conv_bf3w_kernel<false, LDSBN, NH, 1, PL, false, true>), lds_ready_p, 160 * 1024 - 1024)) return -1;
    hipLaunchKernelGGL((conv_bf3w_kernel<false, LDSBN, NH, 1, PL, false, true>), dim3((unsigned)std::min<long long>(blocks, RERUN_GRID), a.groups), dim3(512), lds, s, a, wimg, td);
    return 0;
  }
  hipLaunchKernelGGL((conv_bf3w_kernel<false, LDSBN, NH, 1, PL, H>), dim3((unsigned)blocks, a.groups), dim3(512), lds, s, a, wimg, td);
  return 0;
}
template <class F>
static int with_math(const ConvArgs& a, const WeightImages& im, const uint4* w, F&& launch) {
  using P2 = std::integral_constant<int, 2>;
  if (a.planes == 2 && a.half) return launch(P2{}, std::true_type{}, w + im.half / 16);
  if (a.planes == 2 && im.planes2 != WeightImages::absent) return launch(P2{}, std::false_type{}, w + im.planes2 / 16);
  return launch(std::integral_constant<int, 3>{}, std::false_type{}, w);
}
static int launch_bf3w(const ConvArgs& a, const WeightImages& im, const uint4* w, hipStream_t s) {
  if (a.planes == 2 && a.half && conv_rw_layer(a) && !a.in_planes && !a.out_planes && (!a.sc_in || a.sc_planes)) {
    const int rc = launch_conv_rw(a, w + im.half / 16, s);
    if (rc != -2) return rc;
  }
  return with_math(a, im, w, [&](auto pl, auto h, const uint4* wi) {
    constexpr int PL = decltype(pl)::value;
    constexpr bool H = decltype(h)::value;
    return a.Cout / a.groups == 64 ? launch_bf3w_t<2, PL, H>(a, wi, s) : launch_bf3w_t<1, PL, H>(a, wi, s);
  });
}

template <int NTN, int S, int NB, int TW, int CT, bool C8 = false, int PL = 3, bool H = false>
int launch_bf3_t(const ConvArgs& a, const uint4* wimg, hipStream_t s) {
  constexpr int TB = 128 / TW, TH = TB * NB;
  constexpr int PH = (TH - 1) * S + 3, PW = (TW - 1) * S + 3;
  size_t lds = ((size_t)(C8 ? 3 : 2 * PL) * PH * PW + (size_t)(C8 ? 30 : 18 * PL) * 32 * NTN) * 16;
  if (lds < (CT / 64) * 32 * 32 * sizeof(float)) lds = (CT / 64) * 32 * 32 * sizeof(float);
  static bool lds_ready[64], lds_ready_p[64];
  if (!cpx_dyn_lds_ready(reinterpret_cast<const void*>(conv_bf3_kernel<NTN, S, NB, TW, CT, C8, PL, H>), lds_ready, 160 * 1024 - 1024)) return -1;
  TileDiv td{};
  if (const int rc = fill_tiles(td, (a.Wo + TW - 1) / TW, (a.Ho + TH - 1) / TH, a.N, (a.Cout / a.groups) / (32 * NTN), TILES_PER_LAUNCH)) return rc;
  const long long blocks = td.total;
  if constexpr (PL == 3 && !H) if (a.guard != nullptr) {
    if (!cpx_dyn_lds_ready(reinterpret_cast<const void*>(conv_bf3_kernel<NTN, S, NB, TW, CT, C8, PL, false, true>), lds_ready_p, 160 * 1024 - 1024)) return -1;
    hipLaunchKernelGGL((conv_bf3_kernel<NTN, S, NB, TW, CT, C8, PL, false, true>), dim3((unsigned)std::min<long long>(blocks, RERUN_GRID), a.groups), dim3(CT), lds, s, a, wimg, td);
    return 0;
  }
  hipLaunchKernelGGL((conv_bf3_kernel<NTN, S, NB, TW, CT, C8, PL, H>), dim3((unsigned)blocks, a.groups), dim3(CT), lds, s, a, wimg, td);
  return 0;
}

constexpr int TW_S2 = 16, NB_S2 = 2, CT_S2 = 512;
constexpr int TW_S3 = 16, NB_S3 = 2, CT_S3 = 512, NTN_S3 = 1;
constexpr int NB_S4 = 1, CT_S4 = 256, NTN_S4 = 2;
static_assert(B8_WIMG == (int)WeightImages::C8_HALF_ENTRIES, "conv_block32_kernel<true> and the layout agree on the tap-quad image");

}

static WeightImages images_of(const ConvArgs& a) { return WeightImages::of(conv_shape_of(a)); }
bool conv_bf3_supported(const ConvArgs& a) { return conv_class(conv_shape_of(a)) != ConvClass::Unsupported; }
size_t conv_bf3_weight_bytes(const ConvArgs& a) { return images_of(a).bytes; }
bool conv_bf3_two_planes(const ConvArgs& a) {
  const WeightImages im = images_of(a);
  return im.half != WeightImages::absent && im.cls != ConvClass::C8;
}
bool conv_bf3_can_store_planes(const ConvArgs& a) {
  const ConvClass cls = conv_class(conv_shape_of(a));
  if (cls == ConvClass::Unsupported || cls == ConvClass::Rw3 || (a.Cout / a.groups) % 4 != 0) return false;
  if (cls == ConvClass::Flat && a.stride == 1) return !flat_pays(a, 32, 4 * NB_S4, 256);
  return true;
}
bool conv_bf3_can_load_planes(const ConvArgs& a) {
  return conv_class(conv_shape_of(a)) == ConvClass::Wide && !conv_rw_layer(a);
}
const float* conv_bf3_weight_scales(const ConvArgs& a, const void* wimg) {
  const WeightImages im = images_of(a);
  return im.scales == WeightImages::absent ? nullptr : reinterpret_cast<const float*>(reinterpret_cast<const char*>(wimg) + im.scales);
}
void launch_split_weights(const ConvArgs& a, void* wimg, hipStream_t s) {
  const ConvShape sh = conv_shape_of(a);
  const WeightImages im = WeightImages::of(sh);
  const auto image = [wimg](size_t off) { return reinterpret_cast<uint4*>(reinterpret_cast<char*>(wimg) + off); };
  float* ws = nullptr;
  if (im.scales != WeightImages::absent) {
    ws = reinterpret_cast<float*>(image(im.scales));
    hipLaunchKernelGGL(weight_scales_kernel, dim3((unsigned)((a.Cout + 255) / 256)), dim3(256), 0, s, a.weights, ws, ws + a.Cout,
                       sh.groups, 9 * sh.cin_g, sh.cout_g);
  }
  if (im.cls == ConvClass::C8) {
    hipLaunchKernelGGL(split_weights8_kernel, dim3((unsigned)(((size_t)sh.groups * 10 * sh.cout_g + 255) / 256)), dim3(256), 0, s,
                       a.weights, image(im.planes3), sh.groups, sh.cout_g);
    hipLaunchKernelGGL(split_weights8h_kernel, dim3((unsigned)((sh.groups * 384 + 255) / 256)), dim3(256), 0, s, a.weights,
                       image(im.half), sh.groups, ws);
    return;
  }
  const unsigned grid = (unsigned)(((size_t)sh.groups * (sh.cin_g / 8) * 9 * sh.cout_g + 255) / 256);
  const auto build = [&](int chunk, size_t off, int planes, const float* wscale) {
    if (off == WeightImages::absent) return;
    if (chunk == KW)
      hipLaunchKernelGGL(split_weights32_kernel, dim3(grid), dim3(256), 0, s, a.weights, image(off), sh.groups, sh.cin_g, sh.cout_g, planes, wscale);
    else
      hipLaunchKernelGGL(split_weights_kernel, dim3(grid), dim3(256), 0, s, a.weights, image(off), sh.groups, sh.cin_g, sh.cout_g, planes, wscale);
  };
  build(im.chunk, im.planes3, 3, nullptr);
  build(im.chunk, im.planes2, 2, nullptr);
  build(im.chunk, im.half, 2, ws);
  build(KW, im.rw_half, 2, ws);
}
int launch_conv_bf3(const ConvArgs& a_in, const void* wimg, hipStream_t s) {
  ConvArgs a = a_in;
  const WeightImages im = images_of(a);
  const ConvClass cls = im.cls;
  if (cls == ConvClass::Unsupported) return -2;
  if (cls == ConvClass::Rw3 && !a.half) return launch_conv(a, s);
  if (a.half) {
    if (a.planes != 2 || !conv_bf3_two_planes(a) || a.ovf == nullptr) return -2;
    if (a.in_planes && !conv_bf3_can_load_planes(a)) return -2;
    a.w_scale = conv_bf3_weight_scales(a, wimg);
    a.w_unscale = a.w_scale + a.Cout;
  }
  if ((long long)a.H * a.W >= (1 << 24) || (long long)a.Ho * a.Wo >= (1 << 24) || a.Cin >= (1 << 24) || a.Cout >= (1 << 24)) return -3;
  if (a.in_planes && !a.half) return -2;
  if (a.out_planes && (a.ovf == nullptr || !conv_bf3_can_store_planes(a) || a.residual != nullptr)) return -2;
  const uint4* w = reinterpret_cast<const uint4*>(wimg);
  if (cls == ConvClass::C8) return launch_bf3_t<1, 1, NB_S2, TW_S2, CT_S2, true>(a, w, s);
  if (cls == ConvClass::Rw3) {
    const int rc = launch_conv_rw(a, w + im.half / 16, s);
    return rc == -2 ? launch_conv(a, s) : rc;
  }
  if (cls == ConvClass::Stride2Rw && a.planes == 2 && a.half && !a.out_planes && !a.in_planes) {
    const int rc = launch_conv_rw(a, w + im.rw_half / 16, s);
    if (rc != -2) return rc;
  }
  if (a.stride == 2)
    return with_math(a, im, w, [&](auto pl, auto h, const uint4* wi) {
      return launch_bf3_t<2, 2, 2, 16, 512, false, decltype(pl)::value, decltype(h)::value>(a, wi, s);
    });
  if (cls == ConvClass::Wide) {
    if (a.sc_in && ((a.sc_cin / a.groups) & 3)) return -2;
    return launch_bf3w(a, im, w, s);
  }
  if (a.Cout / a.groups == 32) return launch_bf3_t<1, 1, NB_S2, TW_S2, CT_S2>(a, w, s);
  if (a.Cout / a.groups == 64) return launch_bf3_t<NTN_S3, 1, NB_S3, TW_S3, CT_S3>(a, w, s);
  if (flat_pays(a, 32, 4 * NB_S4, 256)) {
    if (a.planes == 2 && a.half && a.sc_in && a.sc_planes && conv_shortcut_planes_layer(a, a.sc_cin / a.groups) && !a.residual &&
        a.sc_stride >= 1 && a.sc_xscale > 0.0f && (a.sc_H - 1) / a.sc_stride + 1 == a.Ho && (a.sc_W - 1) / a.sc_stride + 1 == a.Wo &&
        (long long)a.sc_H * a.sc_W * a.sc_cin < (1ll << 31))
      return launch_bf3flat_t<2, 256, 2, true, 256, true>(a, w + im.half / 16, s);
    return with_math(a, im, w, [&](auto pl, auto h, const uint4* wi) {
      return launch_bf3flat_t<2, 256, decltype(pl)::value, decltype(h)::value>(a, wi, s);
    });
  }
  return with_math(a, im, w, [&](auto pl, auto h, const uint4* wi) {
    return launch_bf3_t<NTN_S4, 1, NB_S4, 32, CT_S4, false, decltype(pl)::value, decltype(h)::value>(a, wi, s);
  });
}

bool conv_block32_supported(const ConvArgs& a, const ConvArgs& b) {
  const auto plain = [](const ConvArgs& c) {
    return c.ksize == 3 && c.stride == 1 && c.Cout / c.groups == 32 && c.relu && c.pad_top == 1 && c.pad_left == 1 && !c.out_planes &&
           !c.in_planes;
  };
  if (!(plain(a) && plain(b) && a.in_scale && a.in_shift && !a.residual && !a.sc_in && !b.in_scale && !b.out_scale &&
        a.Cout == b.Cin && b.Cin == b.Cout && a.groups == b.groups && a.H == b.H && a.W == b.W && a.N == b.N && a.ovf != nullptr))
    return false;
  if (a.Cin / a.groups == 8)
    return b.residual == nullptr && b.sc_in == a.in && b.sc_w != nullptr && b.sc_cin == a.Cin && b.sc_stride == 1 && b.sc_H == a.H &&
           b.sc_W == a.W;
  return a.Cin == a.Cout && b.residual == a.in && b.sc_in == nullptr;
}
int launch_conv_block32(const ConvArgs& a_in, const ConvArgs& b_in, const void* wimg_a, const void* wimg_b, hipStream_t s) {
  ConvArgs a = a_in, b = b_in;
  if (!conv_block32_supported(a, b)) return -2;
  if ((long long)a.H * a.W >= (1 << 24)) return -3;
  const WeightImages ia = images_of(a), ib = images_of(b);
  if (ia.half == WeightImages::absent || ib.half == WeightImages::absent) return -2;
  a.w_scale = conv_bf3_weight_scales(a, wimg_a);
  a.w_unscale = a.w_scale + a.Cout;
  b.w_scale = conv_bf3_weight_scales(b, wimg_b);
  b.w_unscale = b.w_scale + b.Cout;
  const uint4* wa = reinterpret_cast<const uint4*>(wimg_a) + ia.half / 16;
  const uint4* wb = reinterpret_cast<const uint4*>(wimg_b) + ib.half / 16;
  TileDiv td{};
  if (const int rc = fill_tiles(td, (a.W + W_TW - 1) / W_TW, (a.H + W_TH - 1) / W_TH, a.N, 1, TILES_PERSISTENT)) return rc;
  const bool c8 = a.Cin / a.groups == 8;
  static const bool split_roles = [] {
    const char* e = std::getenv("CPX_BLOCK32_SPLIT");
    return e == nullptr || std::atoi(e) != 0;
  }();
  if (!c8 && split_roles) return launch_conv_block32s(a, b, wa, wb, s);
  const bool c1 = c8 && a.c1_in != nullptr;
  if (c1 && !(a.groups == 2 && a.c1_w != nullptr && a.c1_b != nullptr)) return -2;
  const size_t lds = c8 ? (size_t)(B_R0 + B8_WIMG + B_WIMG) * 16 + 256 + (size_t)2 * B8_NPXP * 16 + (c1 ? (size_t)(B_C1W + 2 * B_C1C) * 4 : 0)
                        : (size_t)(B_R0 + 2 * B_WIMG) * 16 + 256;
  static bool lds_ready[64], lds_ready8[64], lds_ready1[64];
  if (c1 ? !cpx_dyn_lds_ready(reinterpret_cast<const void*>(conv_block32_kernel<true, true>), lds_ready1, 160 * 1024 - 1024)
      : c8 ? !cpx_dyn_lds_ready(reinterpret_cast<const void*>(conv_block32_kernel<true>), lds_ready8, 160 * 1024 - 1024)
           : !cpx_dyn_lds_ready(reinterpret_cast<const void*>(conv_block32_kernel<false>), lds_ready, 160 * 1024 - 1024))
    return -1;
  const int cus = cpx_device_cus();
  if (cus == 0) return -1;
  const char* e = std::getenv("CPX_BLOCK32_GRID");
  const int gx = e ? persistent_grid_x(std::atoi(e), 1, td.total) : persistent_grid_x(cus, a.groups, td.total);
  if (c1) hipLaunchKernelGGL((conv_block32_kernel<true, true>), dim3((unsigned)gx, a.groups), dim3(512), lds, s, a, b, wa, wb, td);
  else if (c8) hipLaunchKernelGGL(conv_block32_kernel<true>, dim3((unsigned)gx, a.groups), dim3(512), lds, s, a, b, wa, wb, td);
  else hipLaunchKernelGGL(conv_block32_kernel<false>, dim3((unsigned)gx, a.groups), dim3(512), lds, s, a, b, wa, wb, td);
  return 0;
}

}
```

classifier-pipeline_amd/csrc/cpx_cnn_rw.hip:

```cpp
#include <hip/hip_runtime.h>

#include <algorithm>
#include <type_traits>

#include "cpx_conv_layout_core.h"
#include "cpx_kernels.h"

namespace cpx {

namespace {

typedef unsigned u32x4 __attribute__((ext_vector_type(4)));
typedef float f32x4 __attribute__((ext_vector_type(4)));
typedef _Float16 f16x2 __attribute__((ext_vector_type(2)));
typedef _Float16 f16x8 __attribute__((ext_vector_type(8)));

template <typename T>
__device__ __forceinline__ const T* at_off(const T* base, unsigned bytes) {
  return reinterpret_cast<const T*>(reinterpret_cast<const char*>(base) + bytes);
}
template <typename T>
__device__ __forceinline__ T* at_off(T* base, unsigned bytes) {
  return reinterpret_cast<T*>(reinterpret_cast<char*>(base) + bytes);
}
__device__ __forceinline__ unsigned pix_off(int y, int x, int W, int C) {
  return __umul24(__umul24((unsigned)y, (unsigned)W) + (unsigned)x, (unsigned)C);
}
__device__ __forceinline__ float relu_bits(float x) { return __int_as_float(max(__float_as_int(x), 0)); }
__device__ __forceinline__ void split_h(float a, float b, unsigned& hi, unsigned& lo) {
  f16x2 v = {(_Float16)a, (_Float16)b};
  hi = __builtin_bit_cast(unsigned, v);
  asm("v_fma_mixlo_f16 %0, %1, 1.0, -%2 op_sel:[0,0,0] op_sel_hi:[0,0,1]" : "=v"(lo) : "v"(a), "v"(hi));
  asm("v_fma_mixhi_f16 %0, %1, 1.0, -%2 op_sel:[0,0,1] op_sel_hi:[0,0,1]" : "+v"(lo) : "v"(b), "v"(hi));
}
__device__ __forceinline__ f32x4 mfma_h(u32x4 w, u32x4 x, f32x4 c) {
  return __builtin_amdgcn_mfma_f32_16x16x32_f16(__builtin_bit_cast(f16x8, w), __builtin_bit_cast(f16x8, x), c, 0, 0, 0);
}

struct RwTiles {
  unsigned long long m_tx, m_ty;
  int tiles_x, tiles_y, total;
};
template <int I, int N, typename F>
__device__ __forceinline__ void static_for(F&& f) {
  if constexpr (I < N) {
    f(std::integral_constant<int, I>{});
    static_for<I + 1, N>(f);
  }
}
__device__ __forceinline__ int div_magic(int n, unsigned long long m) { return (int)(((unsigned long long)n * m) >> 42); }

constexpr int RW_TW = 16;
constexpr int RW_CT = 256;
constexpr int RW_PPI = RW_CT / 8;
constexpr int RW_WC = 64;

template <int S, int NCH, int ROWS>
struct RwGeo {
  static constexpr int PW = 15 * S + 3, PH = (ROWS - 1) * S + 3, NPX = PH * PW;
  static constexpr int NP = (NPX * 8 + RW_CT - 1) / RW_CT;
  static constexpr int NPXP = (NP * RW_PPI + 3) / 4 * 4 + 2;
  static constexpr int BUF = 2 * 2 * NPXP * 2;
  static constexpr int STEPS = 3 * PH;
  static constexpr int CING = 32 * NCH;
  static constexpr size_t LDS = (size_t)2 * BUF * 16 + (size_t)(2 * CING + 3 * RW_WC) * sizeof(float);
};
constexpr int SC_NPXP = 258;
constexpr int SC_ITEMS = 16 * RW_TW * 8 / RW_CT;
constexpr size_t SC_LDS = (size_t)2 * 2 * SC_NPXP * 2 * 16;

template <int S, int NCH, int ROWS, bool BN, bool RES, bool SC = false>
__global__ __launch_bounds__(RW_CT) __attribute__((amdgpu_waves_per_eu(1, 1))) void conv_rw_kernel(ConvArgs a, const uint4* __restrict__ wimg, RwTiles td) {
  using G = RwGeo<S, NCH, ROWS>;
  constexpr int PW = G::PW, NPX = G::NPX, NP = G::NP, NPXP = G::NPXP, BUF = G::BUF, STEPS = G::STEPS, CING = G::CING, PH = G::PH;
  static_assert(!SC || (S == 1 && NCH == 2 && ROWS == 16 && !RES), "the fp16 shortcut is built into the stride-1 form's two-chunk stream");
  if (*a.ovf != 0) return;
  extern __shared__ __attribute__((aligned(16))) uint4 lds4[];
  uint4* s_buf = lds4;
  float* s_bn = reinterpret_cast<float*>(lds4 + 2 * BUF);
  float* s_par = s_bn + 2 * CING;
  uint4* s_sc = reinterpret_cast<uint4*>(s_par + 3 * RW_WC);
  const int tid = threadIdx.x, lane = tid & 63, wave = tid >> 6, i16 = lane & 15, q = lane >> 4;
  const int ct = wave;
  const int cout_g = a.Cout / a.groups, nhalf = cout_g / RW_WC;
  const int g = blockIdx.y / nhalf, half = blockIdx.y - g * nhalf;
  constexpr bool has_bn = BN;

  u32x4 Wr[NCH][9][2];
  {
    const u32x4* wg = reinterpret_cast<const u32x4*>(wimg) + (size_t)g * NCH * 3 * 24 * cout_g + (q * cout_g + half * RW_WC + ct * 16 + i16);
#pragma unroll
    for (int c = 0; c < NCH; ++c)
#pragma unroll
      for (int ky = 0; ky < 3; ++ky)
#pragma unroll
        for (int kx = 0; kx < 3; ++kx)
#pragma unroll
          for (int p = 0; p < 2; ++p) Wr[c][ky * 3 + kx][p] = wg[(size_t)((c * 3 + ky) * 24 + (p * 3 + kx) * 4) * cout_g];
  }
  u32x4 Wsc[2];
  if constexpr (SC) {
    const u32x4* ws = reinterpret_cast<const u32x4*>(a.sc_planes) + (size_t)g * 8 * cout_g + (q * cout_g + half * RW_WC + ct * 16 + i16);
    Wsc[0] = ws[0];
    Wsc[1] = ws[(size_t)4 * cout_g];
  }
  if (tid < CING) {
    const int ci = g * CING + tid;
    s_bn[tid] = has_bn ? a.in_scale[ci] * a.act_scale : a.act_scale;
    s_bn[CING + tid] = has_bn ? a.in_shift[ci] * a.act_scale : 0.0f;
  }
  if (tid < RW_WC) {
    const int ch = g * cout_g + half * RW_WC + tid;
    float os = a.w_unscale[ch] * a.act_unscale;
    if (a.out_scale) os *= a.out_scale[ch];
    float ob = a.out_shift ? a.out_shift[ch] : 0.0f;
    if (a.sc_in && a.sc_bias) ob += a.sc_bias[ch];
    s_par[tid] = os;
    s_par[RW_WC + tid] = ob;
    s_par[2 * RW_WC + tid] = a.w_scale[ch] * a.act_scale;
  }

  const int per_xcd = (td.total + 7) >> 3;
  auto tile_of = [&](int t) { return (t & 7) * per_xcd + (t >> 3); };
  auto decode = [&](int tile, int& n_, int& oy_, int& ox_) {
    int qd = div_magic(tile, td.m_tx);
    ox_ = (tile - qd * td.tiles_x) * RW_TW;
    tile = qd;
    qd = div_magic(tile, td.m_ty);
    oy_ = (tile - qd * td.tiles_y) * ROWS;
    n_ = qd;
  };
  int t = blockIdx.x;
  while (t < 8 * per_xcd && tile_of(t) >= td.total) t += gridDim.x;
  if (t >= 8 * per_xcd) return;
  auto advance = [&](int& n_, int& oy_, int& ox_) {
    t += gridDim.x;
    const bool more = t < 8 * per_xcd && tile_of(t) < td.total;
    if (more) decode(tile_of(t), n_, oy_, ox_);
    return more;
  };
  int n0, oy0, ox0, n1, oy1, ox1, n2, oy2, ox2;
  decode(tile_of(t), n0, oy0, ox0);

  u32x4 pre_p[NP];
  const int q8 = tid & 7;
  int ipos[NP];
#pragma unroll
  for (int i = 0; i < NP; ++i) {
    const int px = min((tid >> 3) + RW_PPI * i, NPX - 1);
    const int py = px / PW;
    ipos[i] = (py << 8) | (px - py * PW);
  }
  const unsigned st_base = (unsigned)((((q8 >> 2) * NPXP + (tid >> 3)) * 4 + (q8 & 3)) * 8);
  f32x4 psc[NCH], psh[NCH];
  const unsigned coff0 = (unsigned)(g * CING + 4 * q8);
  auto med3 = [](int x, int lo, int hi) __attribute__((always_inline)) {
    int r;
    asm("v_med3_i32 %0, %1, %2, %3" : "=v"(r) : "v"(x), "v"(lo), "s"(hi));
    return r;
  };
  const int Hm1 = a.H - 1, Wm1 = a.W - 1;
  auto issue_item = [&](const int i, const int c, const int n_, const int oy_, const int ox_) __attribute__((always_inline)) {
    const float* in_n = a.in + (size_t)n_ * a.H * a.W * a.Cin;
    const int iy = oy_ * S - a.pad_top + (ipos[i] >> 8), ix = ox_ * S - a.pad_left + (ipos[i] & 0xFF);
    const int cy = med3(iy, 0, Hm1), cx = med3(ix, 0, Wm1);
    pre_p[i] = *reinterpret_cast<const u32x4*>(at_off(in_n, (pix_off(cy, cx, a.W, a.Cin) + coff0 + (unsigned)(c * 32)) << 2));
  };
  unsigned hmax = 0u;
  auto pk_max_u16 = [](unsigned x, unsigned y) __attribute__((always_inline)) {
    unsigned r;
    asm("v_pk_max_u16 %0, %1, %2" : "=v"(r) : "v"(x), "v"(y));
    return r;
  };
  auto activate_item = [&](const int i, const int c, const int oy_, const int ox_) __attribute__((always_inline)) {
    float v[4];
#pragma unroll
    for (int j = 0; j < 4; ++j) v[j] = __fmaf_rn(__uint_as_float(pre_p[i][j]), psc[c][j], psh[c][j]);
    if (has_bn) {
#pragma unroll
      for (int j = 0; j < 4; ++j) v[j] = fmaxf(v[j], 0.0f);
    }
    const int iy = oy_ * S - a.pad_top + (ipos[i] >> 8), ix = ox_ * S - a.pad_left + (ipos[i] & 0xFF);
    const bool inside = (unsigned)iy < (unsigned)a.H && (unsigned)ix < (unsigned)a.W;
#pragma unroll
    for (int j = 0; j < 4; ++j) pre_p[i][j] = __float_as_uint(inside ? v[j] : 0.0f);
  };
  auto store_item = [&](const int i, const int bsel) __attribute__((always_inline)) {
    unsigned h0, h1, l0, l1;
    split_h(__uint_as_float(pre_p[i][0]), __uint_as_float(pre_p[i][1]), h0, l0);
    split_h(__uint_as_float(pre_p[i][2]), __uint_as_float(pre_p[i][3]), h1, l1);
    if (has_bn) hmax = pk_max_u16(pk_max_u16(hmax, h0), h1);
    else hmax = pk_max_u16(pk_max_u16(hmax, h0 & 0x7FFF7FFFu), h1 & 0x7FFF7FFFu);
    unsigned char* sp = reinterpret_cast<unsigned char*>(s_buf) + st_base;
    *reinterpret_cast<uint2*>(sp + (bsel * BUF * 16 + i * (RW_PPI * 32))) = make_uint2(h0, h1);
    *reinterpret_cast<uint2*>(sp + (bsel * BUF * 16 + 2 * NPXP * 32 + i * (RW_PPI * 32))) = make_uint2(l0, l1);
  };

  u32x4 pre_s[SC ? SC_ITEMS : 1];
  u32x4 xsh[2], xsl[2];
  const unsigned sc_st_base = (unsigned)((((q8 >> 2) * SC_NPXP + (tid >> 3)) * 4 + (q8 & 3)) * 8);
  const int sc_a_base = ((q >> 1) * SC_NPXP + i16) * 2 + (q & 1);
  auto issue_sc = [&](const int i, const int n_, const int oy_, const int ox_) __attribute__((always_inline)) {
    if constexpr (SC) {
      const float* sc_n = a.sc_in + (size_t)n_ * a.sc_H * a.sc_W * a.sc_cin;
      const int oy = min(oy_ + 2 * i + (tid >> 7), a.Ho - 1), ox = min(ox_ + ((tid >> 3) & 15), a.Wo - 1);
      pre_s[i] = *reinterpret_cast<const u32x4*>(
          at_off(sc_n, (pix_off(oy * a.sc_stride, ox * a.sc_stride, a.sc_W, a.sc_cin) + (unsigned)(g * 32 + 4 * q8)) << 2));
    }
  };
  auto store_sc = [&](const int i) __attribute__((always_inline)) {
    if constexpr (SC) {
      unsigned h0, h1, l0, l1;
      split_h(__uint_as_float(pre_s[i][0]) * a.sc_xscale, __uint_as_float(pre_s[i][1]) * a.sc_xscale, h0, l0);
      split_h(__uint_as_float(pre_s[i][2]) * a.sc_xscale, __uint_as_float(pre_s[i][3]) * a.sc_xscale, h1, l1);
      hmax = pk_max_u16(pk_max_u16(hmax, h0 & 0x7FFF7FFFu), h1 & 0x7FFF7FFFu);
      unsigned char* sp = reinterpret_cast<unsigned char*>(s_sc) + sc_st_base;
      *reinterpret_cast<uint2*>(sp + i * (RW_PPI * 32)) = make_uint2(h0, h1);
      *reinterpret_cast<uint2*>(sp + (2 * SC_NPXP * 32 + i * (RW_PPI * 32))) = make_uint2(l0, l1);
    }
  };

  f32x4 acc[ROWS];
  const int ch_l = g * cout_g + half * RW_WC + ct * 16 + 4 * q;
  auto init_acc = [&]() __attribute__((always_inline)) {
#pragma unroll
    for (int o = 0; o < ROWS; ++o) acc[o] = f32x4{0.0f, 0.0f, 0.0f, 0.0f};
  };
  f32x4 rres[RES ? ROWS : 1];
  auto issue_res = [&](const int o, const int n_, const int oy_, const int ox_) __attribute__((always_inline)) {
    if constexpr (RES) {
      const float* res_n = a.residual + (size_t)n_ * a.Ho * a.Wo * a.Cout;
      const int ox = min(ox_ + i16, a.Wo - 1), oy = min(oy_ + o, a.Ho - 1);
      rres[o] = *reinterpret_cast<const f32x4*>(at_off(res_n, (pix_off(oy, ox, a.Wo, a.Cout) + (unsigned)ch_l) << 2));
    }
  };

  const int a_base = ((q >> 1) * NPXP + S * i16) * 2 + (q & 1);
  constexpr int RW_AHEAD = 3, RW_RING = RW_AHEAD + 1;
  auto compute = [&](auto cc, auto bc, auto&& between) __attribute__((always_inline)) {
    constexpr int C = decltype(cc)::value, B = decltype(bc)::value;
    const uint4* sb = s_buf + B * BUF + a_base;
    u32x4 xh[RW_RING], xl[RW_RING];
    auto frag = [&](auto sc) __attribute__((always_inline)) {
      constexpr int s = decltype(sc)::value;
      constexpr int kx = s / PH, i = s - PH * kx, bf = s % RW_RING;
      xh[bf] = __builtin_bit_cast(u32x4, sb[(i * PW + kx) * 2]);
      xl[bf] = __builtin_bit_cast(u32x4, sb[4 * NPXP + (i * PW + kx) * 2]);
    };
    static_for<0, RW_AHEAD>(frag);
    static_for<0, STEPS>([&](auto sc) __attribute__((always_inline)) {
      constexpr int s = decltype(sc)::value;
      constexpr int kx = s / PH, i = s - PH * kx, bf = s % RW_RING;
      if constexpr (s + RW_AHEAD < STEPS) frag(std::integral_constant<int, s + RW_AHEAD>{});
      static_for<0, 3>([&](auto pc) __attribute__((always_inline)) {
        constexpr int pr = decltype(pc)::value;
        static_for<0, 3>([&](auto rc) __attribute__((always_inline)) {
          constexpr int r = decltype(rc)::value, d = i - r, o = d / S;
          if constexpr (d >= 0 && d % S == 0 && o < ROWS) {
            if constexpr (pr == 0) acc[o] = mfma_h(Wr[C][r * 3 + kx][1], xh[bf], acc[o]);
            if constexpr (pr == 1) acc[o] = mfma_h(Wr[C][r * 3 + kx][0], xl[bf], acc[o]);
            if constexpr (pr == 2) acc[o] = mfma_h(Wr[C][r * 3 + kx][0], xh[bf], acc[o]);
          }
        });
      });
      between(sc);
      __builtin_amdgcn_sched_barrier(0);
    });
  };
  auto unit = [&](auto cc, auto bc, auto ccc, auto cic, auto lastc, const int oyc, const int oxc, const int ni, const int oyi,
                  const int oxi) __attribute__((always_inline)) {
    constexpr int B = decltype(bc)::value, CC = decltype(ccc)::value, CI = decltype(cic)::value;
    constexpr bool LAST = decltype(lastc)::value;
    compute(cc, bc, [&](auto sc) __attribute__((always_inline)) {
      constexpr int s = decltype(sc)::value;
      constexpr int jlo = (s * 3 * NP + STEPS - 1) / STEPS, jhi = ((s + 1) * 3 * NP + STEPS - 1) / STEPS;
      static_for<jlo, (jhi < 3 * NP ? jhi : 3 * NP)>([&](auto jc) __attribute__((always_inline)) {
        constexpr int j = decltype(jc)::value, i = j / 3, k = j % 3;
        if constexpr (k == 0) activate_item(i, CC, oyc, oxc);
        if constexpr (k == 1) store_item(i, B ^ 1);
        if constexpr (k == 2) issue_item(i, CI, ni, oyi, oxi);
      });
      if constexpr (SC && !LAST) {
        constexpr int klo = (s * SC_ITEMS + STEPS - 1) / STEPS, khi = ((s + 1) * SC_ITEMS + STEPS - 1) / STEPS;
        static_for<klo, (khi < SC_ITEMS ? khi : SC_ITEMS)>([&](auto kc) __attribute__((always_inline)) { store_sc(decltype(kc)::value); });
      }
      if constexpr (SC && LAST) {
        if constexpr (s % 3 == 0 && s >= 3 && s / 3 - 1 < ROWS) {
          constexpr int o = s / 3 - 1;
          acc[o] = mfma_h(Wsc[1], xsh[o & 1], acc[o]);
          acc[o] = mfma_h(Wsc[0], xsl[o & 1], acc[o]);
          acc[o] = mfma_h(Wsc[0], xsh[o & 1], acc[o]);
        }
        if constexpr (s % 3 == 0 && s / 3 < ROWS) {
          constexpr int o = s / 3;
          xsh[o & 1] = __builtin_bit_cast(u32x4, s_sc[sc_a_base + o * 2 * RW_TW]);
          xsl[o & 1] = __builtin_bit_cast(u32x4, s_sc[sc_a_base + 4 * SC_NPXP + o * 2 * RW_TW]);
        }
        constexpr int klo = (s * SC_ITEMS + STEPS - 1) / STEPS, khi = ((s + 1) * SC_ITEMS + STEPS - 1) / STEPS;
        static_for<klo, (khi < SC_ITEMS ? khi : SC_ITEMS)>([&](auto kc) __attribute__((always_inline)) { issue_sc(decltype(kc)::value, ni, oyi, oxi); });
      }
      if constexpr (LAST && RES) {
        constexpr int olo = (s * ROWS + STEPS - 1) / STEPS, ohi = ((s + 1) * ROWS + STEPS - 1) / STEPS;
        static_for<olo, (ohi < ROWS ? ohi : ROWS)>([&](auto oc) __attribute__((always_inline)) { issue_res(decltype(oc)::value, n0, oy0, ox0); });
      }
    });
  };

  auto finish = [&](const int n_, const int oy_, const int ox_) __attribute__((always_inline)) {
    const int ox = min(ox_ + i16, a.Wo - 1);
    if (!SC && a.sc_in) {
      const int sc_cg = a.sc_cin / a.groups;
      const float* wsc = a.sc_w + ((size_t)g * sc_cg + q) * cout_g + half * RW_WC + ct * 16 + i16;
      const float ss = s_par[2 * RW_WC + ct * 16 + i16];
      const float* sc_n = a.sc_in + (size_t)n_ * a.sc_H * a.sc_W * a.sc_cin + g * sc_cg + q;
      for (int k4 = 0; k4 < sc_cg; k4 += 4) {
        const float ws = wsc[(size_t)k4 * cout_g] * ss;
#pragma unroll
        for (int o = 0; o < ROWS; ++o) {
          const int oy = min(oy_ + o, a.Ho - 1);
          const float xs = sc_n[((size_t)(oy * a.sc_stride) * a.sc_W + ox * a.sc_stride) * a.sc_cin + k4];
          acc[o] = __builtin_amdgcn_mfma_f32_16x16x4f32(ws, xs, acc[o], 0, 0, 0);
        }
      }
    }
    float* out_n = a.out + (size_t)n_ * a.Ho * a.Wo * a.Cout;
    const f32x4 os = *reinterpret_cast<const f32x4*>(s_par + ct * 16 + 4 * q);
    const f32x4 ob = *reinterpret_cast<const f32x4*>(s_par + RW_WC + ct * 16 + 4 * q);
    const bool xok = ox_ + i16 < a.Wo;
    const unsigned off0 = (pix_off(min(oy_, a.Ho - 1), ox, a.Wo, a.Cout) + (unsigned)ch_l) << 2;
    const unsigned row_bytes = (unsigned)(a.Wo * a.Cout) << 2;
    const bool whole = oy_ + ROWS <= a.Ho;
    auto row = [&](const int o, const bool ok, const unsigned off) __attribute__((always_inline)) {
      f32x4 v;
#pragma unroll
      for (int j = 0; j < 4; ++j) v[j] = __fmaf_rn(acc[o][j], os[j], ob[j]);
      if constexpr (RES) v += rres[o];
      if (a.relu) {
        asm volatile("");
        v.x = relu_bits(v.x); v.y = relu_bits(v.y); v.z = relu_bits(v.z); v.w = relu_bits(v.w);
      }
      if (ok) *reinterpret_cast<f32x4*>(at_off(out_n, off)) = v;
    };
    if (whole) {
#pragma unroll
      for (int o = 0; o < ROWS; ++o) row(o, xok, off0 + (unsigned)o * row_bytes);
    } else {
#pragma unroll
      for (int o = 0; o < ROWS; ++o) row(o, xok && oy_ + o < a.Ho, off0 + (unsigned)min(o, a.Ho - 1 - oy_) * row_bytes);
    }
  };

#pragma unroll
  for (int i = 0; i < NP; ++i) issue_item(i, 0, n0, oy0, ox0);
  __syncthreads();
#pragma unroll
  for (int c = 0; c < NCH; ++c) {
    psc[c] = *reinterpret_cast<const f32x4*>(s_bn + c * 32 + 4 * q8);
    psh[c] = *reinterpret_cast<const f32x4*>(s_bn + CING + c * 32 + 4 * q8);
  }
#pragma unroll
  for (int i = 0; i < NP; ++i) {
    activate_item(i, 0, oy0, ox0);
    store_item(i, 0);
  }
  using I0 = std::integral_constant<int, 0>;
  using I1 = std::integral_constant<int, 1>;
  using Yes = std::integral_constant<bool, true>;
  using No = std::integral_constant<bool, false>;
  if constexpr (NCH == 2) {
#pragma unroll
    for (int i = 0; i < NP; ++i) issue_item(i, 1, n0, oy0, ox0);
    if constexpr (SC) {
#pragma unroll
      for (int i = 0; i < SC_ITEMS; ++i) issue_sc(i, n0, oy0, ox0);
    }
    init_acc();
    for (;;) {
      n1 = n0; oy1 = oy0; ox1 = ox0;
      const bool more = advance(n1, oy1, ox1);
      __syncthreads();
      unit(I0{}, I0{}, I1{}, I0{}, No{}, oy0, ox0, n1, oy1, ox1);
      __syncthreads();
      unit(I1{}, I1{}, I0{}, I1{}, Yes{}, oy1, ox1, n1, oy1, ox1);
      finish(n0, oy0, ox0);
      if (!more) break;
      n0 = n1; oy0 = oy1; ox0 = ox1;
      init_acc();
    }
  } else {
    n1 = n0; oy1 = oy0; ox1 = ox0;
    bool more1 = advance(n1, oy1, ox1);
#pragma unroll
    for (int i = 0; i < NP; ++i) issue_item(i, 0, n1, oy1, ox1);
    init_acc();
    for (;;) {
      n2 = n1; oy2 = oy1; ox2 = ox1;
      bool more2 = more1 && advance(n2, oy2, ox2);
      __syncthreads();
      unit(I0{}, I0{}, I0{}, I0{}, Yes{}, oy1, ox1, n2, oy2, ox2);
      finish(n0, oy0, ox0);
      if (!more1) break;
      n0 = n1; oy0 = oy1; ox0 = ox1; n1 = n2; oy1 = oy2; ox1 = ox2; more1 = more2;
      init_acc();
      n2 = n1; oy2 = oy1; ox2 = ox1;
      more2 = more1 && advance(n2, oy2, ox2);
      __syncthreads();
      unit(I0{}, I1{}, I0{}, I0{}, Yes{}, oy1, ox1, n2, oy2, ox2);
      finish(n0, oy0, ox0);
      if (!more1) break;
      n0 = n1; oy0 = oy1; ox0 = ox1; n1 = n2; oy1 = oy2; ox1 = ox2; more1 = more2;
      init_acc();
    }
  }
  if ((hmax & 0x7FFFu) >= 0x7C00u || ((hmax >> 16) & 0x7FFFu) >= 0x7C00u) atomicOr(a.ovf, 1);
}

__global__ __launch_bounds__(256) void split_shortcut_kernel(const float* __restrict__ w, uint4* __restrict__ out, int groups, int cin_g,
                                                             int cout_g, const float* __restrict__ wscale, float factor) {
  const int nch = cin_g / 32;
  const int total = groups * nch * 4 * cout_g;
  const int idx = blockIdx.x * blockDim.x + threadIdx.x;
  if (idx >= total) return;
  const int col = idx % cout_g;
  int r = idx / cout_g;
  const int qq = r & 3;
  r >>= 2;
  const int chunk = r % nch, g = r / nch;
  const float f = wscale[g * cout_g + col] * factor;
  float v[8];
#pragma unroll
  for (int j = 0; j < 8; ++j) v[j] = w[((size_t)g * cin_g + chunk * 32 + 8 * qq + j) * cout_g + col] * f;
  uint4 hi, lo;
  split_h(v[0], v[1], hi.x, lo.x);
  split_h(v[2], v[3], hi.y, lo.y);
  split_h(v[4], v[5], hi.z, lo.z);
  split_h(v[6], v[7], hi.w, lo.w);
  const size_t base = (size_t)(g * nch + chunk) * 8 * cout_g + (size_t)qq * cout_g + col;
  out[base] = hi;
  out[base + (size_t)4 * cout_g] = lo;
}

}

bool conv_shortcut_planes_layer(const ConvArgs& second, int sc_cin_g) {
  if (conv_rw_kind(second) == 1) return sc_cin_g == 32;
  return second.ksize == 3 && second.stride == 1 && second.groups >= 1 && second.Cin == second.Cout &&
         second.Cout == 128 * second.groups && sc_cin_g == 64;
}
size_t conv_shortcut_image_bytes(int groups, int cin_g, int cout_g) { return (size_t)groups * (cin_g / 32) * 8 * cout_g * 16; }
void launch_split_shortcut(const float* sc_w, void* img, int groups, int cin_g, int cout_g, const float* w_scale, float factor,
                           hipStream_t s) {
  const int total = groups * (cin_g / 32) * 4 * cout_g;
  hipLaunchKernelGGL(split_shortcut_kernel, dim3((unsigned)((total + 255) / 256)), dim3(256), 0, s, sc_w, reinterpret_cast<uint4*>(img),
                     groups, cin_g, cout_g, w_scale, factor);
}

int conv_rw_kind(const ConvArgs& a) { return conv_rw_kind_of(conv_shape_of(a)); }
bool conv_rw_layer(const ConvArgs& a) { return conv_rw_kind(a) == 1; }

namespace {
template <int S, int NCH, int ROWS, bool BN, bool RES, bool SC = false>
int launch_rw_t(const ConvArgs& a, const uint4* wimg, hipStream_t s) {
  using G = RwGeo<S, NCH, ROWS>;
  constexpr size_t LDS = G::LDS + (SC ? SC_LDS : 0);
  static_assert(LDS <= 160 * 1024 - 1024, "two chunk buffers (and the shortcut's operand) must fit the CU's LDS");
  RwTiles td{};
  if (const int rc = fill_tiles(td, (a.Wo + RW_TW - 1) / RW_TW, (a.Ho + ROWS - 1) / ROWS, a.N, TILES_PERSISTENT)) return rc;
  static bool lds_ready[64];
  if (!cpx_dyn_lds_ready(reinterpret_cast<const void*>(conv_rw_kernel<S, NCH, ROWS, BN, RES, SC>), lds_ready, 160 * 1024 - 1024)) return -1;
  const int cus = cpx_device_cus();
  if (cus == 0) return -1;
  const int ny = a.groups * ((a.Cout / a.groups) / RW_WC);
  const int gx = persistent_grid_x(cus, ny, td.total);
  hipLaunchKernelGGL((conv_rw_kernel<S, NCH, ROWS, BN, RES, SC>), dim3((unsigned)gx, (unsigned)ny), dim3(RW_CT), LDS, s, a, wimg, td);
  return 0;
}
}

int launch_conv_rw(const ConvArgs& a, const void* wimg, hipStream_t s) {
  const int kind = conv_rw_kind(a);
  if (!kind || !a.half || a.planes != 2 || a.ovf == nullptr || a.in_planes || a.out_planes) return -2;
  if ((long long)a.H * a.W >= (1 << 24) || (long long)a.Ho * a.Wo >= (1 << 24)) return -3;
  if (a.sc_in && ((a.sc_cin / a.groups) & 3)) return -2;
  const uint4* wi = reinterpret_cast<const uint4*>(wimg);
  const bool bn = a.in_scale != nullptr, res = a.residual != nullptr;
  if (kind == 1) {
    if (a.pad_top != 1 || a.pad_left != 1 || a.H != a.Ho || a.W != a.Wo) return -2;
    if (a.sc_in && a.sc_planes) {
      if (bn || res || !conv_shortcut_planes_layer(a, a.sc_cin / a.groups) || a.sc_stride < 1 || !(a.sc_xscale > 0.0f) ||
          (a.sc_H - 1) / a.sc_stride + 1 != a.Ho || (a.sc_W - 1) / a.sc_stride + 1 != a.Wo)
        return -2;
      if ((long long)a.sc_H * a.sc_W >= (1 << 24) || (long long)a.sc_H * a.sc_W * a.sc_cin >= (1ll << 30)) return -3;
      return launch_rw_t<1, 2, 16, false, false, true>(a, wi, s);
    }
    if (bn && res) return launch_rw_t<1, 2, 16, true, true>(a, wi, s);
    if (bn) return launch_rw_t<1, 2, 16, true, false>(a, wi, s);
    if (res) return launch_rw_t<1, 2, 16, false, true>(a, wi, s);
    return launch_rw_t<1, 2, 16, false, false>(a, wi, s);
  }
  if (res || a.sc_in || a.pad_top < 0 || a.pad_top > 1 || a.pad_left < 0 || a.pad_left > 1) return -2;
  if (kind == 2) return bn ? launch_rw_t<2, 1, 8, true, false>(a, wi, s) : launch_rw_t<2, 1, 8, false, false>(a, wi, s);
  return bn ? launch_rw_t<3, 2, 4, true, false>(a, wi, s) : launch_rw_t<3, 2, 4, false, false>(a, wi, s);
}

}
```

classifier-pipeline_amd/csrc/cpx_internal.h:

```cpp
#pragma once
#include <hip/hip_runtime.h>

#include <map>
#include <string>
#include <vector>

#include "cpx.h"
#include "cpx_kernels.h"

struct cpx_cnn;
struct cpx_mog2;
struct cpx_graph;
void cnn_free(cpx_cnn* c);
void graph_free(cpx_graph* g);
void mog2_free(cpx_mog2* m);

struct DeviceBuffer {
  void* p = nullptr;
  size_t bytes = 0;
  DeviceBuffer() = default;
  DeviceBuffer(const DeviceBuffer&) = delete;
  DeviceBuffer& operator=(const DeviceBuffer&) = delete;
  int grow(cpx_handle* h, size_t need, const char* what);
  void release() {
    if (p) hipFree(p);
    p = nullptr;
    bytes = 0;
  }
  template <class T>
  T* as() const { return static_cast<T*>(p); }
};

struct cpx_handle {
  int device = 0;
  cpx_config cfg{};
  hipStream_t stream = nullptr;
  std::string err;
  DeviceBuffer ws;
  DeviceBuffer wtab_dev, wthr_dev;
  int wtab_len = 0;
  std::vector<double> wtab_host;
  DeviceBuffer nlm_lut_dev;
  DeviceBuffer sched;
  struct ConvEv { int key; double flops; hipEvent_t e0, e1; };
  std::vector<ConvEv> conv_events;
  bool conv_timing = false;
  DeviceBuffer ws_assoc;
  hipEvent_t ev0 = nullptr, ev1 = nullptr;
  int last_launches = 0;
  bool timing_valid = false;
  hipStream_t stream2 = nullptr;
  bool state_packed = false;
  bool packed_state_ok = true;
  bool fuse_conv1 = true;
  bool medians_pending = false;
  hipEvent_t ev_median = nullptr;
  bool track_per_step = false;
  std::vector<struct cpx_cnn*> cnns;
  std::vector<struct cpx_mog2*> mog2s;
  std::vector<struct cpx_graph*> graphs;
  DeviceBuffer graph_arena;
  int stream_frames = -1;
  int stream_assoc_frames = -1;
  bool stream_filt_state = false;
  int last_B = 0;
  struct StagedBackground { std::vector<uint16_t> bg, kcnt; double average; };
  std::map<int, StagedBackground> staged_bg;
  int cnn_math = CPX_CNN_MATH_FP16X2;
  bool fuse_shortcut = true;
  bool shortcut_fp16 = true;
  DeviceBuffer bf3_scratch;
  DeviceBuffer cnn_arena;
  DeviceBuffer cnn_ovf;
  int block_fusion = 2;
  DeviceBuffer ir_scratch;
  DeviceBuffer ir_bitmap;
};

inline int fail(cpx_handle* h, int code, const char* what, hipError_t e = hipSuccess) {
  if (h) {
    h->err = what;
    if (e != hipSuccess) {
      h->err += ": ";
      h->err += hipGetErrorString(e);
    }
  }
  return code;
}

#define CPX_HIP(h, call)                                            \
  do {                                                              \
    hipError_t _e = (call);                                         \
    if (_e != hipSuccess) return fail((h), CPX_ERR_HIP, #call, _e); \
  } while (0)

#define CPX_ENTER(h)                           \
  do {                                         \
    CPX_HIP((h), hipSetDevice((h)->device));   \
    (void)hipGetLastError();                   \
  } while (0)

inline int DeviceBuffer::grow(cpx_handle* h, size_t need, const char* what) {
  if (need <= bytes) return CPX_OK;
  if (p) CPX_HIP(h, hipStreamSynchronize(h->stream));
  release();
  const hipError_t e = hipMalloc(&p, need);
  if (e != hipSuccess) {
    p = nullptr;
    (void)hipGetLastError();
    return fail(h, CPX_ERR_NOMEM, what, e);
  }
  bytes = need;
  return CPX_OK;
}

inline size_t align_up(size_t v, size_t a) { return (v + a - 1) / a * a; }
```

classifier-pipeline_amd/csrc/cpx_kernels.h:

```cpp
#pragma once
#include <hip/hip_runtime.h>
#include <stddef.h>
#include <stdint.h>

#include "cpx.h"

#ifndef CPX_TRACK_THREADS
#define CPX_TRACK_THREADS 768
#endif
#ifndef CPX_TRACK_CHUNKS
#define CPX_TRACK_CHUNKS 7
#endif
#ifndef CPX_TRACK_LDS_COMPONENTS
#define CPX_TRACK_LDS_COMPONENTS 256
#endif
#ifndef CPX_TRACK_MIN_WAVES_PER_SIMD
#define CPX_TRACK_MIN_WAVES_PER_SIMD 6
#endif

namespace cpx {

typedef cpx_component Component;
typedef cpx_frame_info FrameInfo;

// ... 14 lines not shown
};

struct FrameCarry {
  Red1 R;
  int avg_change, mn, mx, ithr;
  float thresh, median;
  int pad;
  double bg_avg_in;
};

struct TrackArgs {
  int W, H, edge, window, cap_out;
  int flags;
  double background_thresh;
  double weight_add;
  const uint16_t* frames;
  const int* clip_first;
  const int* proc_off;
  const int* proc_idx;
  const int* proc_ffc;
  const int* order;
  const double* wtab;
  int wtab_len;
  const uint32_t* wthr;
  int nlm_flip;
  double* bgavg;
  uint16_t* bg;
  uint32_t* wsum;
  uint16_t* kcnt;
  int packed_state;
  float* filt_state;
  ClipState* cstate;
  unsigned char* u8_state;
  FrameCarry* carry;
  const int* nlm_lut;
  uint32_t* big_stat;
  Component* comps_out;
  FrameInfo* info_out;
  int32_t* labels_out;
  float* filtered_out;
};

struct ActiveTrack;
struct ScoreRec;
struct AssocResume {
  int n_active, n_tracks, next_id, status;
};
struct AssocArgs {
  int B, cap;
  int t_begin;
  int fresh;
  AssocResume* resume;
  cpx_track_params params;
  const int* clip_first;
  const int* proc_off;
  const int* proc_idx;
  const int* proc_ffc;
  const Component* comps;
  const FrameInfo* info;
  cpx_region* pool;
  cpx_track_record* tracks;
  int* n_tracks;
  int* status;
  cpx_region* regions_out;
  int* region_counts;
  ActiveTrack* active;
  cpx_region* regs;
  ScoreRec* scores;
  unsigned char* used;
};
void launch_assoc(const AssocArgs& a, hipStream_t s);
struct FinalArgs {
  int B, square_width, max_frames;
  cpx_filter_params params;
  const int* clip_first;
  const int* proc_off;
  const int* proc_idx;
  const int* proc_ffc;
  const cpx_region* pool;
  const cpx_track_record* tracks;
  const int* n_tracks;
  cpx_track_summary* summaries;
  int* counts;
  double* scratch_d;
  float* scratch_f;
  const int* prefix;
  cpx_region_ref* refs;
  int* track_offsets;
  cpx_crop_req* reqs;
  int* sample_track;
  int* track_clip;
};
void launch_finalize(const FinalArgs& a, hipStream_t s);
void launch_plan(const FinalArgs& a, hipStream_t s);
void launch_counts_prefix(const int* counts, int B, int* prefix, hipStream_t s);
size_t assoc_active_bytes();
size_t assoc_score_bytes();

struct ClassifyArgs {
  int W, H, crop_x, crop_y, crop_w, crop_h;
  int frame_size, square_width;
  int limits_flags;
  const uint16_t* frames;
  const float* filtered;
  const FrameInfo* info;
  const cpx_region_ref* refs;
  const int* track_offsets;
  cpx_track_limits* limits;
  const cpx_crop_req* reqs;
  float* out;
};
struct AggregateArgs {
  int n_samples, n_tracks, n_labels, fp_index, square_width;
  const float* probs;
  const int* sample_track;
  const cpx_crop_req* reqs;
  float* scores;
  int* best;
};
void launch_aggregate(const AggregateArgs& a, hipStream_t s);
void launch_limits(const ClassifyArgs& a, int n_tracks, hipStream_t s);
int launch_crop(const ClassifyArgs& a, int n_reqs, hipStream_t s);

struct ConvArgs {
  int N, H, W, Cin, Cout, groups, ksize, stride, relu;
  int Ho, Wo, pad_top, pad_left;
  const float* in;
  float* out;
  const float* weights;
  const float* in_scale;
  const float* in_shift;
  const float* out_scale;
  const float* out_shift;
  const float* residual;
  const float* sc_in;
  const float* sc_w;
  const float* sc_bias;
  int sc_H, sc_W, sc_cin, sc_stride;
  const void* sc_planes;
  float sc_xscale;
  const float* c1_in;
  const float* c1_w;
  const float* c1_b;
  int planes;
  int half;
  float act_scale, act_unscale;
  const float* w_scale;
  const float* w_unscale;
  int* ovf;
  const int* guard;
  int out_planes, in_planes;
  float out_act_scale;
};
struct HeadArgs {
  int N, HW, C, L;
  int n_hidden, activation;
  int hidden_sizes[CPX_HEAD_MAX_HIDDEN];
  const float* in;
  const float* bn_scale;
  const float* bn_shift;
  const float* hidden_w[CPX_HEAD_MAX_HIDDEN];
  const float* hidden_b[CPX_HEAD_MAX_HIDDEN];
  const float* dense_w;
  const float* dense_b;
  float* logits;
  float* probs;
};
int launch_conv(const ConvArgs& a, hipStream_t s);
bool conv_bf3_supported(const ConvArgs& a);
size_t conv_bf3_weight_bytes(const ConvArgs& a);
bool conv_bf3_two_planes(const ConvArgs& a);
bool conv_bf3_can_store_planes(const ConvArgs& a);
bool conv_bf3_can_load_planes(const ConvArgs& a);
void launch_split_weights(const ConvArgs& a, void* wimg, hipStream_t s);
int launch_conv_bf3(const ConvArgs& a, const void* wimg, hipStream_t s);
bool conv_block32_supported(const ConvArgs& a, const ConvArgs& b);
int launch_conv_block32(const ConvArgs& a, const ConvArgs& b, const void* wimg_a, const void* wimg_b, hipStream_t s);
int launch_conv_block32s(const ConvArgs& a, const ConvArgs& b, const void* wa, const void* wb, hipStream_t s);
int conv_rw_kind(const ConvArgs& a);
bool conv_rw_layer(const ConvArgs& a);
int launch_conv_rw(const ConvArgs& a, const void* wimg, hipStream_t s);
bool conv_shortcut_planes_layer(const ConvArgs& second, int sc_cin_g);
size_t conv_shortcut_image_bytes(int groups, int cin_g, int cout_g);
void launch_split_shortcut(const float* sc_w, void* img, int groups, int cin_g, int cout_g, const float* w_scale, float factor,
                           hipStream_t s);
const float* conv_bf3_weight_scales(const ConvArgs& a, const void* wimg);
void launch_head(const HeadArgs& a, hipStream_t s);
void launch_count_overflow(int* ovf, int n_words, hipStream_t s);

struct CptvArgs {
  int W, H;
  const unsigned char* payload;
  const long long* frame_offsets;
  const int* bit_widths;
  const int* clip_offsets;
  uint16_t* frames_out;
};
int launch_cptv_unpack(const CptvArgs& a, int B, hipStream_t s);

struct CptvInflateArgs {
  int B;
  const unsigned char* in;
  const cpx_cptv_file* files;
  unsigned char* out;
  cpx_cptv_frame_slot* slots;
  unsigned char* header;
  cpx_cptv_file_result* results;
};
int launch_cptv_inflate(const CptvInflateArgs& a, hipStream_t s);

struct CptvGatherArgs {
  const cpx_cptv_frame_slot* slots;
  const long long* slot_offsets;
  const int* clip_offsets;
  long long* frame_offsets;
  int* bit_widths;
  cpx_cptv_frame_slot* slots_out;
};
int launch_cptv_gather(const CptvGatherArgs& a, int B, hipStream_t s);

struct ThumbArgs {
  int W, H, chain_cap;
  int max_w, max_h;
  const uint16_t* frames;
  const int32_t* labels;
  const cpx_frame_info* info;
  const cpx_region_ref* refs;
  cpx_thumb_stat* out;
};
int launch_thumb(const ThumbArgs& a, int n_refs, hipStream_t s);

struct TracklessArgs {
  int W, H, frame, background;
  const uint16_t* frames;
  int32_t* out;
  const int32_t* pairs;
  int n;
};
int launch_trackless(const TracklessArgs& a, hipStream_t s);

struct IrArgs {
  int W, H, threshold, max_components;
  const unsigned char* images;
  cpx_component* comps;
  int32_t* counts;
  int32_t* status;
  int32_t* labels;
  unsigned char* slots;
  size_t slot_bytes;
  uint32_t* slot_bitmap;
  int n_slots;
};
int launch_ir_detect(const IrArgs& a, int n_frames, hipStream_t s);
struct IrVarArgs {
  int W, H, n;
  const unsigned char* cur;
  const unsigned char* prev;
  const int* rects;
  double* out;
};
void launch_ir_delta_variance(const IrVarArgs& a, hipStream_t s);
struct IrMergeArgs {
  int W, H, n, cap_in, cap_out;
  int frame_number, out_stride;
  const cpx_component* comps;
  const int* counts;
  const unsigned char* cur;
  const unsigned char* prev;
  cpx_component* out_comps;
  cpx_frame_info* out_info;
  int* status;
};
void launch_ir_merge(const IrMergeArgs& a, hipStream_t s);
void launch_ir_resize_area(const unsigned char* src, unsigned char* dst, int n, int W, int H, int f, hipStream_t s);
struct IrStatsArgs {
  int n, pixels, vec16;
  const unsigned char* frames;
  const unsigned char* masks;
  unsigned int* hist;
  cpx_ir_frame_stats* out;
};
void launch_ir_frame_stats(const IrStatsArgs& a, hipStream_t s);
int ir_supported(int W, int H);
size_t ir_slot_bytes(int W, int H);

struct Mog2Args {
  size_t n;
  float alphaT, alpha1, prune;
  float var_threshold, background_ratio, var_threshold_gen, var_init, var_min, var_max;
  const unsigned char* frames;
  float* weight;
  float* var;
  float* mean;
  unsigned char* modes;
  unsigned char* mask;
};
void launch_mog2_apply(const Mog2Args& a, hipStream_t s);
void launch_mog2_background(const Mog2Args& a, unsigned char* out, hipStream_t s);

struct GraphView {
  float* p;
  int H, W, C, cstride;
  size_t sample_stride;
};
struct GraphOpArgs {
  int kind;
  int N;
  GraphView in0, in1, out;
  int kh, kw, stride_h, stride_w, pad_top, pad_left;
  int act;
  int n_map, map[4];
  float param;
  const float* weights;
  const float* scale;
  const float* shift;
  int in0_int8;
};
void launch_graph_op(const GraphOpArgs& a, hipStream_t s);
constexpr int GRAPH_CONV_KC = 16;
constexpr int GRAPH_CONV_CO = 32;
void launch_graph_q8_op(const GraphOpArgs& a, hipStream_t s);
constexpr int GRAPH_CONV_Q8_KC = 32;
void launch_graph_h2_op(const GraphOpArgs& a, hipStream_t s);
constexpr int GRAPH_CONV_H2_KC = 32;
void launch_graph_dw_op(const GraphOpArgs& a, hipStream_t s);
void launch_graph_i8_op(const GraphOpArgs& a, hipStream_t s);
// ... 38 lines not shown
```

Before: 3.165 million.

## Hand over fp16 planes in a block16 layout between flat and rw convs

Adds a second planes layout (PLANES_BLOCK16) so a block's first convolution can write its activations directly as split fp16 hi/lo planes in 16-channel blocks, which the rw kernel and flat bf3 kernel can then load (the rw kernel through a DMA-style direct path). This is meant to remove the f32 store, the reload and the per-load split work between the two convs of a residual block. When this layout is used, the exact-split reruns are deferred until after both convs, adding extra launches and kernel template variants. Off by default only for layers where a cost heuristic says the handover does not pay. A debug plan print is also added.

```diff
diff --git a/classifier-pipeline_amd/csrc/cpx_api.cpp b/classifier-pipeline_amd/csrc/cpx_api.cpp
--- a/classifier-pipeline_amd/csrc/cpx_api.cpp
+++ b/classifier-pipeline_amd/csrc/cpx_api.cpp
@@ -155,6 +155,7 @@
   if (const char* env = std::getenv("CPX_TRACK_PER_STEP")) h->track_per_step = std::atoi(env) != 0;
   if (const char* env = std::getenv("CPX_CNN_FUSE_SHORTCUT")) h->fuse_shortcut = std::atoi(env) != 0;
   if (const char* env = std::getenv("CPX_CNN_SHORTCUT_FP16")) h->shortcut_fp16 = std::atoi(env) != 0;
+  if (const char* env = std::getenv("CPX_CNN_PLANES_HANDOVER")) h->planes_handover = std::min(std::max(std::atoi(env), 0), 2);
   if (const char* env = std::getenv("CPX_CNN_BLOCK_FUSION")) h->block_fusion = std::min(std::max(std::atoi(env), 0), 2);
   if (const char* env = std::getenv("CPX_CNN_MATH")) {
     if (!std::strcmp(env, "f32")) h->cnn_math = CPX_CNN_MATH_F32;
diff --git a/classifier-pipeline_amd/csrc/cpx_api_cnn.cpp b/classifier-pipeline_amd/csrc/cpx_api_cnn.cpp
--- a/classifier-pipeline_amd/csrc/cpx_api_cnn.cpp
+++ b/classifier-pipeline_amd/csrc/cpx_api_cnn.cpp
@@ -54,10 +54,11 @@
   float act_scale = 1.0f;
   bool keep_flag = false;
   int word = 0;
-  bool out_planes = false;
+  int out_planes = 0;
   float out_act_scale = 1.0f;
-  bool in_planes = false;
+  int in_planes = 0;
   bool rerun_only = false;
+  bool skip_rerun = false;
 };
 constexpr int OVF_WORDS = 2 + 3 * CPX_WRRESNET_MAX_BLOCKS;
 static int ensure_ovf_word(cpx_handle* h) {
@@ -181,14 +182,14 @@
     }
     first.ovf = word;
     if (planes_out) {
-      first.out_planes = 1;
+      first.out_planes = k.out_planes;
       first.out_act_scale = k.out_act_scale;
     }
     rc = cpx::launch_conv_bf3(first, split_weights, h->stream);
   }
   a.guard = word;
   if (split) {
-    if (rc == 0) rc = cpx::launch_conv_bf3(a, split_weights, h->stream);
+    if (rc == 0 && !(route == ConvRoute::Fp16Pair && k.skip_rerun)) rc = cpx::launch_conv_bf3(a, split_weights, h->stream);
     if (rc == -3) {
       if (fuse) return fail(h, CPX_ERR_UNSUPPORTED, "conv_run: batch too large for the fused-shortcut kernel (split the call)");
       rc = cpx::launch_conv(a, h->stream);
@@ -231,6 +232,7 @@
   int stride, H, W, Ho, Wo, c_in, f;
   int word;
   BlockForm form;
+  int planes;
   Shortcut shortcut;
   bool shortcut_fp16;
   Conv1 conv1;
@@ -327,9 +329,12 @@
   const bool c1_inside = one_launch && most == Fusion::BlockAndConv1 && k == 0 && first8 && h->fuse_conv1 && g == 2 &&
                          p.in_channels == 2 && p.filters[0] == 16;
   bp.conv1 = k != 0 ? Conv1::NotHere : c1_inside ? Conv1::InsideBlock : Conv1::InFront;
-  const bool planes = fp16 && whole_groups && cpx::conv_bf3_can_store_planes(first) && cpx::conv_bf3_two_planes(second) &&
-                      cpx::conv_bf3_can_load_planes(second);
+  const int layout = cpx::conv_bf3_load_planes(second, bp.shortcut == Shortcut::FusedIntoSecond && !bp.shortcut_fp16);
+  const bool wanted = h->planes_handover == 2 || (h->planes_handover == 1 && cpx::conv_bf3_planes_pay(first, second, layout));
+  const bool planes = fp16 && wanted && whole_groups && layout != cpx::PLANES_NONE &&
+                      cpx::conv_bf3_two_planes(second) && cpx::conv_bf3_can_store_planes(first, layout);
   bp.form = one_launch ? BlockForm::OneLaunch : planes ? BlockForm::PlanesPair : BlockForm::Separate;
+  bp.planes = bp.form == BlockForm::PlanesPair ? layout : cpx::PLANES_NONE;
   return bp;
 }
 
@@ -351,7 +356,7 @@
   return run_layer(fw, d, hf);
 }
 
-static int run_layers(const Forward& fw, const BlockPlan& bp, bool planes, bool rerun_only) {
+static int run_layers(const Forward& fw, const BlockPlan& bp, int planes, bool rerun_only) {
   const BlockLayers l = block_layers(fw, bp);
   const float* act_scale = fw.cnn->act_scale[bp.st][bp.d];
   const conv_half hf = forward_half(bp.word, rerun_only);
@@ -361,10 +366,17 @@
   ha.out_act_scale = act_scale[1];
   hb.act_scale = act_scale[1];
   hb.in_planes = planes;
+  const bool late_reruns = planes == cpx::PLANES_BLOCK16 && !rerun_only;
+  ha.skip_rerun = hb.skip_rerun = late_reruns;
+  const conv_fuse* fuse = bp.shortcut == Shortcut::FusedIntoSecond ? &l.fuse : nullptr;
   if (int rc = run_layer(fw, l.a, ha)) return rc;
   if (bp.shortcut == Shortcut::OwnLaunch)
     if (int rc = run_layer(fw, l.sc, hf)) return rc;
-  return run_layer(fw, l.b, hb, bp.shortcut == Shortcut::FusedIntoSecond ? &l.fuse : nullptr);
+  if (int rc = run_layer(fw, l.b, hb, fuse)) return rc;
+  if (!late_reruns) return CPX_OK;
+  const conv_half rerun = forward_half(bp.word, true);
+  if (int rc = run_layer(fw, l.a, rerun)) return rc;
+  return run_layer(fw, l.b, rerun, fuse);
 }
 
 static int run_one_launch(const Forward& fw, const BlockPlan& bp, int* declined) {
@@ -383,7 +395,7 @@
   if (int rc = timer.commit((bp.c_in / g) * 10000 + 32 * 10 + 4, flops)) return rc;
   if (bp.conv1 == Conv1::InsideBlock)
     if (int rc = run_conv1(fw, forward_half(bp.word, true))) return rc;
-  return run_layers(fw, bp, false, true);
+  return run_layers(fw, bp, cpx::PLANES_NONE, true);
 }
 
 static int downgrade(const Forward& fw, BlockPlan* bp, int declined) {
@@ -405,7 +417,7 @@
     if (!declined) return CPX_OK;
     if (int rc = downgrade(fw, &bp, declined)) return rc;
   }
-  return run_layers(fw, bp, bp.form == BlockForm::PlanesPair, false);
+  return run_layers(fw, bp, bp.planes, false);
 }
 
 static int update_shortcut_images(cpx_cnn* cnn) {
@@ -482,6 +494,15 @@
     plan[k] = plan_block(fw, k, hh, ww, Fusion::BlockAndConv1);
     hh = plan[k].Ho;
     ww = plan[k].Wo;
+  }
+  if (std::getenv("CPX_CNN_DEBUG_PLAN")) {
+    std::fprintf(stderr, "cpx_cnn_forward: N = %d, plan", N);
+    for (int k = 0; k < n_blocks; ++k) {
+      std::fprintf(stderr, " %d.%d:", plan[k].st + 2, plan[k].d);
+      if (plan[k].form == BlockForm::PlanesPair) std::fprintf(stderr, "p%d", plan[k].planes);
+      else std::fprintf(stderr, "%s", plan[k].form == BlockForm::OneLaunch ? "1" : "s");
+    }
+    std::fprintf(stderr, "\n");
   }
   for (int k = 0; k < n_blocks; ++k) {
     if (int brc = run_block(fw, plan[k])) return brc;
diff --git a/classifier-pipeline_amd/csrc/cpx_cnn_bf3.hip b/classifier-pipeline_amd/csrc/cpx_cnn_bf3.hip
--- a/classifier-pipeline_amd/csrc/cpx_cnn_bf3.hip
+++ b/classifier-pipeline_amd/csrc/cpx_cnn_bf3.hip
@@ -548,6 +548,13 @@
       for (int i = 0; i < NP; ++i) {
         const int iy = iy0 + item_py[i], ix = ix0 + item_px[i];
         const bool inside = iy >= 0 && iy < a.H && ix >= 0 && ix < a.W;
+        if (H && a.in_planes) {
+          const u32x4 zero = u32x4{0u, 0u, 0u, 0u};
+          u32x4* sp4 = reinterpret_cast<u32x4*>(s_patch);
+          sp4[0 * 2 * NPXC + item_e[i]] = inside ? __builtin_bit_cast(u32x4, pre_p[i][0]) : zero;
+          sp4[1 * 2 * NPXC + item_e[i]] = inside ? __builtin_bit_cast(u32x4, pre_p[i][1]) : zero;
+          continue;
+        }
         float v[8];
 #pragma unroll
         for (int j = 0; j < 8; ++j) v[j] = pre_p[i][j >> 2][j & 3];
@@ -606,9 +613,11 @@
 #pragma unroll
       for (int i = 0; i < NP; ++i) {
         const int cy = min(max(iy0 + item_py[i], 0), a.H - 1), cx = min(max(ix0 + item_px[i], 0), a.W - 1);
-        const unsigned soff = (pix_off(cy, cx, a.W, a.Cin) + (unsigned)(cn + 8 * my_h)) << 2;
+        const bool pl_in = H && a.in_planes;
+        const unsigned soff = pl_in ? (pix_off(cy, cx, a.W, a.Cin) << 2) + (unsigned)(((cn >> 4) << 6) + (my_h << 4))
+                                    : (pix_off(cy, cx, a.W, a.Cin) + (unsigned)(cn + 8 * my_h)) << 2;
         pre_p[i][0] = *reinterpret_cast<const f32x4*>(at_off(in_n, soff));
-        pre_p[i][1] = *reinterpret_cast<const f32x4*>(at_off(in_n, soff + 16));
+        pre_p[i][1] = *reinterpret_cast<const f32x4*>(at_off(in_n, soff + (pl_in ? 32u : 16u)));
       }
       const u32x4* wc = reinterpret_cast<const u32x4*>(wg + (size_t)(cc + 1) * (18 * PL) * cout_g);
 #pragma unroll
@@ -732,7 +741,11 @@
     const int ch = ch0 + t * 32 + (lane & 31);
     float os = a.out_scale ? a.out_scale[ch] : 1.0f;
     if (H) os *= a.w_unscale[ch] * a.act_unscale;
-    const float ob = (a.out_shift ? a.out_shift[ch] : 0.0f) + (a.sc_in && a.sc_bias ? a.sc_bias[ch] : 0.0f);
+    float ob = (a.out_shift ? a.out_shift[ch] : 0.0f) + (a.sc_in && a.sc_bias ? a.sc_bias[ch] : 0.0f);
+    if (H && a.out_planes) {
+      os *= a.out_act_scale;
+      ob *= a.out_act_scale;
+    }
 #pragma unroll
     for (int r = 0; r < 16; ++r) {
       const int i = (r & 3) + 8 * (r >> 2) + 4 * (lane >> 5);
@@ -741,7 +754,27 @@
     __builtin_amdgcn_fence(__ATOMIC_RELEASE, "wavefront");
     __builtin_amdgcn_wave_barrier();
     __builtin_amdgcn_fence(__ATOMIC_ACQUIRE, "wavefront");
-    if (res_n) {
+    if (H && a.out_planes) {
+      float vmax = 0.0f;
+#pragma unroll
+      for (int it = 0; it < 4; ++it) {
+        const int f = it * 64 + lane;
+        const int i = f >> 3, c4 = f & 7;
+        const int p = p0 + wave * 32 + i;
+        if (p < M) {
+          f32x4 v = *reinterpret_cast<const f32x4*>(s_tile + i * 32 + 4 * c4);
+          v.x = relu_bits(v.x); v.y = relu_bits(v.y); v.z = relu_bits(v.z); v.w = relu_bits(v.w);
+          vmax = fmaxf(fmaxf(fmaxf(v.x, v.y), fmaxf(v.z, v.w)), vmax);
+          unsigned h0, h1, l0, l1;
+          split_pair2_h(v.x, v.y, h0, l0);
+          split_pair2_h(v.z, v.w, h1, l1);
+          const unsigned o = ((__umul24((unsigned)p, (unsigned)a.Cout) + (unsigned)(ch0 + t * 32)) << 2) + (unsigned)(64 * (c4 >> 2) + 8 * (c4 & 3));
+          *reinterpret_cast<uint2*>(at_off(out_n, o)) = make_uint2(h0, h1);
+          *reinterpret_cast<uint2*>(at_off(out_n, o + 32u)) = make_uint2(l0, l1);
+        }
+      }
+      if (vmax > F16_MAX) atomicOr(a.ovf, 1);
+    } else if (res_n) {
 #pragma unroll
       for (int it = 0; it < 4; ++it) {
         const int f = it * 64 + lane;
@@ -1842,10 +1875,11 @@
   return launch(std::integral_constant<int, 3>{}, std::false_type{}, w);
 }
 static int launch_bf3w(const ConvArgs& a, const WeightImages& im, const uint4* w, hipStream_t s) {
-  if (a.planes == 2 && a.half && conv_rw_layer(a) && !a.in_planes && !a.out_planes && (!a.sc_in || a.sc_planes)) {
+  if (a.planes == 2 && a.half && conv_rw_layer(a) && a.in_planes != PLANES_QUAD && a.out_planes != PLANES_QUAD && (!a.sc_in || a.sc_planes)) {
     const int rc = launch_conv_rw(a, w + im.half / 16, s);
     if (rc != -2) return rc;
   }
+  if (a.in_planes == PLANES_BLOCK16 || a.out_planes == PLANES_BLOCK16) return -2;
   return with_math(a, im, w, [&](auto pl, auto h, const uint4* wi) {
     constexpr int PL = decltype(pl)::value;
     constexpr bool H = decltype(h)::value;
@@ -1887,14 +1921,24 @@
   const WeightImages im = images_of(a);
   return im.half != WeightImages::absent && im.cls != ConvClass::C8;
 }
-bool conv_bf3_can_store_planes(const ConvArgs& a) {
+static bool flat_planes_layer(const ConvArgs& a) {
+  return conv_class(conv_shape_of(a)) == ConvClass::Flat && a.stride == 1 && a.Cin / a.groups % 32 == 0 && flat_pays(a, 32, 4 * NB_S4, 256);
+}
+bool conv_bf3_can_store_planes(const ConvArgs& a, int layout) {
   const ConvClass cls = conv_class(conv_shape_of(a));
-  if (cls == ConvClass::Unsupported || cls == ConvClass::Rw3 || (a.Cout / a.groups) % 4 != 0) return false;
+  if (layout == PLANES_BLOCK16) return conv_rw_kind(a) != 0 || flat_planes_layer(a);
+  if (layout != PLANES_QUAD || cls == ConvClass::Unsupported || cls == ConvClass::Rw3 || (a.Cout / a.groups) % 4 != 0) return false;
   if (cls == ConvClass::Flat && a.stride == 1) return !flat_pays(a, 32, 4 * NB_S4, 256);
   return true;
 }
-bool conv_bf3_can_load_planes(const ConvArgs& a) {
-  return conv_class(conv_shape_of(a)) == ConvClass::Wide && !conv_rw_layer(a);
+bool conv_bf3_planes_pay(const ConvArgs& first, const ConvArgs& second, int layout) {
+  return layout == PLANES_QUAD || (layout == PLANES_BLOCK16 && flat_planes_layer(first) && flat_planes_layer(second));
+}
+int conv_bf3_load_planes(const ConvArgs& a, bool sc_f32) {
+  if (flat_planes_layer(a)) return PLANES_BLOCK16;
+  if (conv_class(conv_shape_of(a)) != ConvClass::Wide) return PLANES_NONE;
+  if (conv_rw_layer(a)) return sc_f32 ? PLANES_NONE : PLANES_BLOCK16;
+  return PLANES_QUAD;
 }
 const float* conv_bf3_weight_scales(const ConvArgs& a, const void* wimg) {
   const WeightImages im = images_of(a);
@@ -1938,22 +1982,25 @@
   if (cls == ConvClass::Rw3 && !a.half) return launch_conv(a, s);
   if (a.half) {
     if (a.planes != 2 || !conv_bf3_two_planes(a) || a.ovf == nullptr) return -2;
-    if (a.in_planes && !conv_bf3_can_load_planes(a)) return -2;
+    if (a.in_planes && a.in_planes != conv_bf3_load_planes(a, a.sc_in && !a.sc_planes)) return -2;
     a.w_scale = conv_bf3_weight_scales(a, wimg);
     a.w_unscale = a.w_scale + a.Cout;
   }
   if ((long long)a.H * a.W >= (1 << 24) || (long long)a.Ho * a.Wo >= (1 << 24) || a.Cin >= (1 << 24) || a.Cout >= (1 << 24)) return -3;
   if (a.in_planes && !a.half) return -2;
-  if (a.out_planes && (a.ovf == nullptr || !conv_bf3_can_store_planes(a) || a.residual != nullptr)) return -2;
+  if (a.out_planes && (a.ovf == nullptr || !conv_bf3_can_store_planes(a, a.out_planes) || a.residual != nullptr)) return -2;
+  const bool chunk32 = a.in_planes == PLANES_BLOCK16 || a.out_planes == PLANES_BLOCK16;
+  if (chunk32 && !(a.half && a.planes == 2 && (conv_rw_kind(a) || flat_planes_layer(a)))) return -2;
+  if (a.out_planes == PLANES_BLOCK16 && (!a.relu || a.sc_in)) return -2;
   const uint4* w = reinterpret_cast<const uint4*>(wimg);
   if (cls == ConvClass::C8) return launch_bf3_t<1, 1, NB_S2, TW_S2, CT_S2, true>(a, w, s);
   if (cls == ConvClass::Rw3) {
     const int rc = launch_conv_rw(a, w + im.half / 16, s);
-    return rc == -2 ? launch_conv(a, s) : rc;
-  }
-  if (cls == ConvClass::Stride2Rw && a.planes == 2 && a.half && !a.out_planes && !a.in_planes) {
+    return rc == -2 && !chunk32 ? launch_conv(a, s) : rc;
+  }
+  if (cls == ConvClass::Stride2Rw && a.planes == 2 && a.half && a.out_planes != PLANES_QUAD && !a.in_planes) {
     const int rc = launch_conv_rw(a, w + im.rw_half / 16, s);
-    if (rc != -2) return rc;
+    if (rc != -2 || chunk32) return rc;
   }
   if (a.stride == 2)
     return with_math(a, im, w, [&](auto pl, auto h, const uint4* wi) {
diff --git a/classifier-pipeline_amd/csrc/cpx_cnn_rw.hip b/classifier-pipeline_amd/csrc/cpx_cnn_rw.hip
--- a/classifier-pipeline_amd/csrc/cpx_cnn_rw.hip
+++ b/classifier-pipeline_amd/csrc/cpx_cnn_rw.hip
@@ -68,12 +68,15 @@
 constexpr int SC_NPXP = 258;
 constexpr int SC_ITEMS = 16 * RW_TW * 8 / RW_CT;
 constexpr size_t SC_LDS = (size_t)2 * 2 * SC_NPXP * 2 * 16;
-
-template <int S, int NCH, int ROWS, bool BN, bool RES, bool SC = false>
+__device__ unsigned rw_zero16[4];
+
+template <int S, int NCH, int ROWS, bool BN, bool RES, bool SC = false, int IN = 0>
 __global__ __launch_bounds__(RW_CT) __attribute__((amdgpu_waves_per_eu(1, 1))) void conv_rw_kernel(ConvArgs a, const uint4* __restrict__ wimg, RwTiles td) {
   using G = RwGeo<S, NCH, ROWS>;
   constexpr int PW = G::PW, NPX = G::NPX, NP = G::NP, NPXP = G::NPXP, BUF = G::BUF, STEPS = G::STEPS, CING = G::CING, PH = G::PH;
   static_assert(!SC || (S == 1 && NCH == 2 && ROWS == 16 && !RES), "the fp16 shortcut is built into the stride-1 form's two-chunk stream");
+  static_assert(!IN || (S == 1 && !BN), "planes are handed to a block's second convolution: stride 1, no prologue");
+  constexpr bool OUT = !IN && !RES && !SC;
   if (*a.ovf != 0) return;
   extern __shared__ __attribute__((aligned(16))) uint4 lds4[];
   uint4* s_buf = lds4;
@@ -115,6 +118,10 @@
     if (a.out_scale) os *= a.out_scale[ch];
     float ob = a.out_shift ? a.out_shift[ch] : 0.0f;
     if (a.sc_in && a.sc_bias) ob += a.sc_bias[ch];
+    if (OUT && a.out_planes) {
+      os *= a.out_act_scale;
+      ob *= a.out_act_scale;
+    }
     s_par[tid] = os;
     s_par[RW_WC + tid] = ob;
     s_par[2 * RW_WC + tid] = a.w_scale[ch] * a.act_scale;
@@ -147,11 +154,12 @@
   int ipos[NP];
 #pragma unroll
   for (int i = 0; i < NP; ++i) {
-    const int px = min((tid >> 3) + RW_PPI * i, NPX - 1);
+    const int px = min((IN == 2 ? lane >> 1 : tid >> 3) + RW_PPI * i, NPX - 1);
     const int py = px / PW;
     ipos[i] = (py << 8) | (px - py * PW);
   }
-  const unsigned st_base = (unsigned)((((q8 >> 2) * NPXP + (tid >> 3)) * 4 + (q8 & 3)) * 8);
+  const unsigned st_base = IN ? (unsigned)((((((q8 >> 1) & 1) * 2 + (q8 >> 2)) * NPXP + (tid >> 3)) * 2 + (q8 & 1)) * 16)
+                              : (unsigned)((((q8 >> 2) * NPXP + (tid >> 3)) * 4 + (q8 & 3)) * 8);
   f32x4 psc[NCH], psh[NCH];
   const unsigned coff0 = (unsigned)(g * CING + 4 * q8);
   auto med3 = [](int x, int lo, int hi) __attribute__((always_inline)) {
@@ -163,16 +171,43 @@
   auto issue_item = [&](const int i, const int c, const int n_, const int oy_, const int ox_) __attribute__((always_inline)) {
     const float* in_n = a.in + (size_t)n_ * a.H * a.W * a.Cin;
     const int iy = oy_ * S - a.pad_top + (ipos[i] >> 8), ix = ox_ * S - a.pad_left + (ipos[i] & 0xFF);
+    if constexpr (IN) {
+      const bool inside = (unsigned)iy < (unsigned)a.H && (unsigned)ix < (unsigned)a.W;
+      const u32x4* src = reinterpret_cast<const u32x4*>(at_off(in_n, (pix_off(iy, ix, a.W, a.Cin) + coff0 + (unsigned)(c * 32)) << 2));
+      pre_p[i] = *(inside ? src : reinterpret_cast<const u32x4*>(rw_zero16));
+      return;
+    }
     const int cy = med3(iy, 0, Hm1), cx = med3(ix, 0, Wm1);
     pre_p[i] = *reinterpret_cast<const u32x4*>(at_off(in_n, (pix_off(cy, cx, a.W, a.Cin) + coff0 + (unsigned)(c * 32)) << 2));
   };
+  static_assert(IN != 2 || (NPXP >= NP * RW_PPI && 4 * NP * 64 >= NPX * 8), "four waves x NP wave-instructions cover the patch inside the regions");
+  const int wave_u = __builtin_amdgcn_readfirstlane(wave);
+  const unsigned dma_src = (unsigned)(g * CING) * 4u + (unsigned)((wave & 1) * 64 + (wave >> 1) * 32 + (lane & 1) * 16);
+  auto dma_item = [&](const int i, const int c, const int bsel, const int n_, const int oy_, const int ox_) __attribute__((always_inline)) {
+    if constexpr (IN == 2) {
+      const float* in_n = a.in + (size_t)n_ * a.H * a.W * a.Cin;
+      const int iy = oy_ * S - a.pad_top + (ipos[i] >> 8), ix = ox_ * S - a.pad_left + (ipos[i] & 0xFF);
+      bool inside = (unsigned)iy < (unsigned)a.H && (unsigned)ix < (unsigned)a.W;
+      if (RW_PPI * (i + 1) > NPX) inside = inside && (lane >> 1) + RW_PPI * i < NPX;
+      const void* src = at_off(reinterpret_cast<const char*>(in_n), (pix_off(iy, ix, a.W, a.Cin) << 2) + dma_src + (unsigned)(c * 128));
+      src = inside ? src : reinterpret_cast<const void*>(rw_zero16);
+      uint4* dst = s_buf + bsel * BUF + (wave_u * NPXP + RW_PPI * i) * 2;
+      __builtin_amdgcn_global_load_lds(reinterpret_cast<const __attribute__((address_space(1))) void*>(reinterpret_cast<size_t>(src)),
+                                       reinterpret_cast<__attribute__((address_space(3))) void*>((unsigned)reinterpret_cast<size_t>(dst)), 16, 0, 0);
+    }
+  };
+  auto dma_wait = [&]() __attribute__((always_inline)) {
+    if constexpr (IN == 2) asm volatile("s_waitcnt vmcnt(0)" ::: "memory");
+  };
   unsigned hmax = 0u;
+  float vmaxf = 0.0f;
   auto pk_max_u16 = [](unsigned x, unsigned y) __attribute__((always_inline)) {
     unsigned r;
     asm("v_pk_max_u16 %0, %1, %2" : "=v"(r) : "v"(x), "v"(y));
     return r;
   };
   auto activate_item = [&](const int i, const int c, const int oy_, const int ox_) __attribute__((always_inline)) {
+    if constexpr (IN) return;
     float v[4];
 #pragma unroll
     for (int j = 0; j < 4; ++j) v[j] = __fmaf_rn(__uint_as_float(pre_p[i][j]), psc[c][j], psh[c][j]);
@@ -186,6 +221,10 @@
     for (int j = 0; j < 4; ++j) pre_p[i][j] = __float_as_uint(inside ? v[j] : 0.0f);
   };
   auto store_item = [&](const int i, const int bsel) __attribute__((always_inline)) {
+    if constexpr (IN) {
+      *reinterpret_cast<u32x4*>(reinterpret_cast<unsigned char*>(s_buf) + st_base + (bsel * BUF * 16 + i * (RW_PPI * 32))) = pre_p[i];
+      return;
+    }
     unsigned h0, h1, l0, l1;
     split_h(__uint_as_float(pre_p[i][0]), __uint_as_float(pre_p[i][1]), h0, l0);
     split_h(__uint_as_float(pre_p[i][2]), __uint_as_float(pre_p[i][3]), h1, l1);
@@ -273,13 +312,21 @@
     constexpr bool LAST = decltype(lastc)::value;
     compute(cc, bc, [&](auto sc) __attribute__((always_inline)) {
       constexpr int s = decltype(sc)::value;
-      constexpr int jlo = (s * 3 * NP + STEPS - 1) / STEPS, jhi = ((s + 1) * 3 * NP + STEPS - 1) / STEPS;
-      static_for<jlo, (jhi < 3 * NP ? jhi : 3 * NP)>([&](auto jc) __attribute__((always_inline)) {
-        constexpr int j = decltype(jc)::value, i = j / 3, k = j % 3;
-        if constexpr (k == 0) activate_item(i, CC, oyc, oxc);
-        if constexpr (k == 1) store_item(i, B ^ 1);
-        if constexpr (k == 2) issue_item(i, CI, ni, oyi, oxi);
-      });
+      if constexpr (IN == 2) {
+        constexpr int DS = STEPS / 2;
+        constexpr int jlo = (s * NP + DS - 1) / DS, jhi = ((s + 1) * NP + DS - 1) / DS;
+        static_for<(jlo < NP ? jlo : NP), (jhi < NP ? jhi : NP)>([&](auto jc) __attribute__((always_inline)) {
+          dma_item(decltype(jc)::value, CC, B ^ 1, LAST ? ni : n0, oyc, oxc);
+        });
+      } else {
+        constexpr int jlo = (s * 3 * NP + STEPS - 1) / STEPS, jhi = ((s + 1) * 3 * NP + STEPS - 1) / STEPS;
+        static_for<jlo, (jhi < 3 * NP ? jhi : 3 * NP)>([&](auto jc) __attribute__((always_inline)) {
+          constexpr int j = decltype(jc)::value, i = j / 3, k = j % 3;
+          if constexpr (k == 0) activate_item(i, CC, oyc, oxc);
+          if constexpr (k == 1) store_item(i, B ^ 1);
+          if constexpr (k == 2) issue_item(i, CI, ni, oyi, oxi);
+        });
+      }
       if constexpr (SC && !LAST) {
         constexpr int klo = (s * SC_ITEMS + STEPS - 1) / STEPS, khi = ((s + 1) * SC_ITEMS + STEPS - 1) / STEPS;
         static_for<klo, (khi < SC_ITEMS ? khi : SC_ITEMS)>([&](auto kc) __attribute__((always_inline)) { store_sc(decltype(kc)::value); });
@@ -327,7 +374,8 @@
     const f32x4 os = *reinterpret_cast<const f32x4*>(s_par + ct * 16 + 4 * q);
     const f32x4 ob = *reinterpret_cast<const f32x4*>(s_par + RW_WC + ct * 16 + 4 * q);
     const bool xok = ox_ + i16 < a.Wo;
-    const unsigned off0 = (pix_off(min(oy_, a.Ho - 1), ox, a.Wo, a.Cout) + (unsigned)ch_l) << 2;
+    const unsigned off0 = ((pix_off(min(oy_, a.Ho - 1), ox, a.Wo, a.Cout) + (unsigned)ch_l) << 2) +
+                          (OUT && a.out_planes ? (unsigned)((2 * (q & 1) + (q >> 1) - q) * 16) : 0u);
     const unsigned row_bytes = (unsigned)(a.Wo * a.Cout) << 2;
     const bool whole = oy_ + ROWS <= a.Ho;
     auto row = [&](const int o, const bool ok, const unsigned off) __attribute__((always_inline)) {
@@ -339,7 +387,20 @@
         asm volatile("");
         v.x = relu_bits(v.x); v.y = relu_bits(v.y); v.z = relu_bits(v.z); v.w = relu_bits(v.w);
       }
-      if (ok) *reinterpret_cast<f32x4*>(at_off(out_n, off)) = v;
+      if (OUT && a.out_planes) {
+        unsigned h0, h1, l0, l1;
+        split_h(v.x, v.y, h0, l0);
+        split_h(v.z, v.w, h1, l1);
+        const bool odd = (q & 1) != 0;
+        const unsigned r0 = (unsigned)__shfl_xor((int)(odd ? h0 : l0), 16), r1 = (unsigned)__shfl_xor((int)(odd ? h1 : l1), 16);
+        if (ok) {
+          if constexpr (S == 3) vmaxf = fmaxf(fmaxf(fmaxf(v.x, v.y), fmaxf(v.z, v.w)), vmaxf);
+          else hmax = pk_max_u16(pk_max_u16(hmax, h0), h1);
+          *reinterpret_cast<u32x4*>(at_off(out_n, off)) = odd ? u32x4{r0, r1, l0, l1} : u32x4{h0, h1, r0, r1};
+        }
+      } else if (ok) {
+        *reinterpret_cast<f32x4*>(at_off(out_n, off)) = v;
+      }
     };
     if (whole) {
 #pragma unroll
@@ -351,25 +412,33 @@
   };
 
 #pragma unroll
-  for (int i = 0; i < NP; ++i) issue_item(i, 0, n0, oy0, ox0);
+  for (int i = 0; i < NP; ++i) {
+    if constexpr (IN == 2) dma_item(i, 0, 0, n0, oy0, ox0);
+    else issue_item(i, 0, n0, oy0, ox0);
+  }
+  dma_wait();
   __syncthreads();
 #pragma unroll
   for (int c = 0; c < NCH; ++c) {
     psc[c] = *reinterpret_cast<const f32x4*>(s_bn + c * 32 + 4 * q8);
     psh[c] = *reinterpret_cast<const f32x4*>(s_bn + CING + c * 32 + 4 * q8);
   }
-#pragma unroll
-  for (int i = 0; i < NP; ++i) {
-    activate_item(i, 0, oy0, ox0);
-    store_item(i, 0);
+  if constexpr (IN != 2) {
+#pragma unroll
+    for (int i = 0; i < NP; ++i) {
+      activate_item(i, 0, oy0, ox0);
+      store_item(i, 0);
+    }
   }
   using I0 = std::integral_constant<int, 0>;
   using I1 = std::integral_constant<int, 1>;
   using Yes = std::integral_constant<bool, true>;
   using No = std::integral_constant<bool, false>;
   if constexpr (NCH == 2) {
-#pragma unroll
-    for (int i = 0; i < NP; ++i) issue_item(i, 1, n0, oy0, ox0);
+    if constexpr (IN != 2) {
+#pragma unroll
+      for (int i = 0; i < NP; ++i) issue_item(i, 1, n0, oy0, ox0);
+    }
     if constexpr (SC) {
 #pragma unroll
       for (int i = 0; i < SC_ITEMS; ++i) issue_sc(i, n0, oy0, ox0);
@@ -378,8 +447,14 @@
     for (;;) {
       n1 = n0; oy1 = oy0; ox1 = ox0;
       const bool more = advance(n1, oy1, ox1);
+      dma_wait();
       __syncthreads();
+      if constexpr (IN == 2 && SC) {
+#pragma unroll
+        for (int i = 0; i < SC_ITEMS; ++i) asm volatile("" : "+v"(pre_s[i]));
+      }
       unit(I0{}, I0{}, I1{}, I0{}, No{}, oy0, ox0, n1, oy1, ox1);
+      dma_wait();
       __syncthreads();
       unit(I1{}, I1{}, I0{}, I1{}, Yes{}, oy1, ox1, n1, oy1, ox1);
       finish(n0, oy0, ox0);
@@ -412,6 +487,8 @@
       init_acc();
     }
   }
+  dma_wait();
+  if (S == 3 && vmaxf > 65504.0f) atomicOr(a.ovf, 1);
   if ((hmax & 0x7FFFu) >= 0x7C00u || ((hmax >> 16) & 0x7FFFu) >= 0x7C00u) atomicOr(a.ovf, 1);
 }
 
@@ -459,7 +536,11 @@
 bool conv_rw_layer(const ConvArgs& a) { return conv_rw_kind(a) == 1; }
 
 namespace {
-template <int S, int NCH, int ROWS, bool BN, bool RES, bool SC = false>
+#ifndef CPX_RW_IN_FORM
+#define CPX_RW_IN_FORM 2
+#endif
+constexpr int RW_IN_FORM = CPX_RW_IN_FORM;
+template <int S, int NCH, int ROWS, bool BN, bool RES, bool SC = false, int IN = 0>
 int launch_rw_t(const ConvArgs& a, const uint4* wimg, hipStream_t s) {
   using G = RwGeo<S, NCH, ROWS>;
   constexpr size_t LDS = G::LDS + (SC ? SC_LDS : 0);
@@ -467,23 +548,26 @@
   RwTiles td{};
   if (const int rc = fill_tiles(td, (a.Wo + RW_TW - 1) / RW_TW, (a.Ho + ROWS - 1) / ROWS, a.N, TILES_PERSISTENT)) return rc;
   static bool lds_ready[64];
-  if (!cpx_dyn_lds_ready(reinterpret_cast<const void*>(conv_rw_kernel<S, NCH, ROWS, BN, RES, SC>), lds_ready, 160 * 1024 - 1024)) return -1;
+  if (!cpx_dyn_lds_ready(reinterpret_cast<const void*>(conv_rw_kernel<S, NCH, ROWS, BN, RES, SC, IN>), lds_ready, 160 * 1024 - 1024)) return -1;
   const int cus = cpx_device_cus();
   if (cus == 0) return -1;
   const int ny = a.groups * ((a.Cout / a.groups) / RW_WC);
   const int gx = persistent_grid_x(cus, ny, td.total);
-  hipLaunchKernelGGL((conv_rw_kernel<S, NCH, ROWS, BN, RES, SC>), dim3((unsigned)gx, (unsigned)ny), dim3(RW_CT), LDS, s, a, wimg, td);
+  hipLaunchKernelGGL((conv_rw_kernel<S, NCH, ROWS, BN, RES, SC, IN>), dim3((unsigned)gx, (unsigned)ny), dim3(RW_CT), LDS, s, a, wimg, td);
   return 0;
 }
 }
 
 int launch_conv_rw(const ConvArgs& a, const void* wimg, hipStream_t s) {
   const int kind = conv_rw_kind(a);
-  if (!kind || !a.half || a.planes != 2 || a.ovf == nullptr || a.in_planes || a.out_planes) return -2;
+  if (!kind || !a.half || a.planes != 2 || a.ovf == nullptr || a.in_planes == PLANES_QUAD || a.out_planes == PLANES_QUAD) return -2;
   if ((long long)a.H * a.W >= (1 << 24) || (long long)a.Ho * a.Wo >= (1 << 24)) return -3;
   if (a.sc_in && ((a.sc_cin / a.groups) & 3)) return -2;
   const uint4* wi = reinterpret_cast<const uint4*>(wimg);
   const bool bn = a.in_scale != nullptr, res = a.residual != nullptr;
+  const bool pin = a.in_planes != 0, pout = a.out_planes != 0;
+  if (pout && (!a.relu || res || a.sc_in || pin)) return -2;
+  if (pin && (kind != 1 || bn || !(res || (a.sc_in && a.sc_planes)))) return -2;
   if (kind == 1) {
     if (a.pad_top != 1 || a.pad_left != 1 || a.H != a.Ho || a.W != a.Wo) return -2;
     if (a.sc_in && a.sc_planes) {
@@ -491,8 +575,9 @@
           (a.sc_H - 1) / a.sc_stride + 1 != a.Ho || (a.sc_W - 1) / a.sc_stride + 1 != a.Wo)
         return -2;
       if ((long long)a.sc_H * a.sc_W >= (1 << 24) || (long long)a.sc_H * a.sc_W * a.sc_cin >= (1ll << 30)) return -3;
-      return launch_rw_t<1, 2, 16, false, false, true>(a, wi, s);
-    }
+      return pin ? launch_rw_t<1, 2, 16, false, false, true, RW_IN_FORM>(a, wi, s) : launch_rw_t<1, 2, 16, false, false, true>(a, wi, s);
+    }
+    if (pin) return a.sc_in ? -2 : launch_rw_t<1, 2, 16, false, true, false, RW_IN_FORM>(a, wi, s);
     if (bn && res) return launch_rw_t<1, 2, 16, true, true>(a, wi, s);
     if (bn) return launch_rw_t<1, 2, 16, true, false>(a, wi, s);
     if (res) return launch_rw_t<1, 2, 16, false, true>(a, wi, s);
diff --git a/classifier-pipeline_amd/csrc/cpx_internal.h b/classifier-pipeline_amd/csrc/cpx_internal.h
--- a/classifier-pipeline_amd/csrc/cpx_internal.h
+++ b/classifier-pipeline_amd/csrc/cpx_internal.h
@@ -68,6 +68,7 @@
   std::map<int, StagedBackground> staged_bg;
   int cnn_math = CPX_CNN_MATH_FP16X2;
   bool fuse_shortcut = true;
+  int planes_handover = 1;
   bool shortcut_fp16 = true;
   DeviceBuffer bf3_scratch;
   DeviceBuffer cnn_arena;
diff --git a/classifier-pipeline_amd/csrc/cpx_kernels.h b/classifier-pipeline_amd/csrc/cpx_kernels.h
--- a/classifier-pipeline_amd/csrc/cpx_kernels.h
+++ b/classifier-pipeline_amd/csrc/cpx_kernels.h
@@ -190,6 +190,7 @@
   int out_planes, in_planes;
   float out_act_scale;
 };
+enum { PLANES_NONE = 0, PLANES_QUAD = 1, PLANES_BLOCK16 = 2 };
 struct HeadArgs {
   int N, HW, C, L;
   int n_hidden, activation;
@@ -208,8 +209,9 @@
 bool conv_bf3_supported(const ConvArgs& a);
 size_t conv_bf3_weight_bytes(const ConvArgs& a);
 bool conv_bf3_two_planes(const ConvArgs& a);
-bool conv_bf3_can_store_planes(const ConvArgs& a);
-bool conv_bf3_can_load_planes(const ConvArgs& a);
+int conv_bf3_load_planes(const ConvArgs& a, bool sc_f32);
+bool conv_bf3_can_store_planes(const ConvArgs& a, int layout);
+bool conv_bf3_planes_pay(const ConvArgs& first, const ConvArgs& second, int layout);
 void launch_split_weights(const ConvArgs& a, void* wimg, hipStream_t s);
 int launch_conv_bf3(const ConvArgs& a, const void* wimg, hipStream_t s);
 bool conv_block32_supported(const ConvArgs& a, const ConvArgs& b);
```

After: 3.161 million, median of 2. No clear change (-0.1%).
